# Skylarking/MARL

Measured on AMD Instinct MI355X. Metric: env_steps_per_sec, higher is better.
Workload: dtype f32 (bf16x6 split products, fp32 accumulate)

## Files before the change

### include/marl_hip.h

```cpp
#ifndef MARL_HIP_H
#define MARL_HIP_H
#include <stddef.h>
#ifdef __cplusplus
extern "C" {
#endif

typedef struct {
  const float* p0; long ld0; int k0;
  const float* p1; long ld1; int k1;
  const int* idx; int nhot; int hot_w;
  int nid;
  const float* m0; long ldm0;
  long rpe0, bs0, off0;
  long rpei, bsi, offi;
  const int* emap0;
} marl_src_t;

typedef struct {
  int groups;
  long gs_x0, gs_x1, gs_w, gs_b, gs_y, gs_m0;
} marl_group_t;

typedef struct {
  const float *fc1_w, *fc1_b;
  const float *w_ih, *w_hh;
  const float *b_ih, *b_hh;
  const float *fc2_w, *fc2_b;
  int H;
} marl_agent_weights_t;

int marl_linear(const marl_src_t* x, const float* W, long ldw, int w_kmajor, const float* bias,
                float* Y, long ldy, int M, int N, int K, int act, float beta,
                const marl_group_t* grp, void* stream);
int marl_linear_wgrad(const float* dY, long lddy, const float* Yact, long ldya, const marl_src_t* x,
                      float* dW, long lddw, float* db, int M, int N, int K, int flags,
                      const marl_group_t* grp, float* ws, size_t ws_bytes, void* stream);
size_t marl_linear_wgrad_workspace(int M, int N, int K, int groups);
int marl_wgrad_slabs(int M);

int marl_agent_unroll_fwd(const marl_agent_weights_t* w, const float* obs, long obs_bs, int obs_t0,
                          const int* ufed, long u_bs, int u_t0, const int* ep_len, const int* ep_map,
                          const float* h0, float* q, float* hs, float* h_last, float* saved, int B, int T,
                          int N, int O, int A, int last_action, int reuse_network, int cu_budget,
                          float* gi_out, const float* gi_in, void* stream);
int marl_agent_unroll_reuse_supported(int B, int T, int N, int O, int A, int cu_budget);

typedef struct {
  float *w_ih, *w_hh;
  float *b_ih, *b_hh;
  float *fc2_w, *fc2_b;
} marl_agent_grads_t;

size_t marl_agent_bwd_workspace(int B, int N, int A);
int marl_agent_unroll_bwd(const marl_agent_weights_t* w, const float* dq, const int* dq_idx,
                          const float* dq_val, const int* dq_idx2, const float* dq_val2, int dq_gdiv, const float* dhs,
                          const float* saved, const float* hs, float* dxp, float* dh0,
                          const marl_agent_grads_t* g, float* ws, size_t ws_bytes,
                          int B, int T, int N, int A, void* stream);

int marl_q_gather(const float* q, const int* idx, const float* avail, float mask_val, float* out,
                  long rows, int A, void* stream);
int marl_q_masked_max(const float* q, const float* avail, float mask_val, float* out_max, int* out_arg,
                      long rows, int A, void* stream);
int marl_q_double_select(const float* q_sel, const float* q_val, const float* avail, float mask_val,
                         float* out_val, int* out_arg, long rows, int A, void* stream);
int marl_q_scatter(float* dq, const int* idx1, const float* g1, const int* idx2, const float* g2,
                   long rows, int A, int gdiv, void* stream);
int marl_vec_add(const float* a, const float* b, float* out, long n, void* stream);
int marl_agent_sum(const float* in, long ld_in, float* out, long ld_out, long rows, int N, int D, void* stream);
int marl_agent_bcast(const float* in, long ld_in, float* out, long ld_out, long rows, int N, int D, int accumulate,
                     void* stream);

int marl_qmix_mix_fwd(const float* hy, long ldh, const float* b2, const float* w22, const float* b22, const float* q,
                      float* q_tot, long rows, int N, int E, void* stream);
int marl_qmix_mix_bwd(const float* hy, long ldh, const float* q, const float* dq_tot, const float* w22, float* dhy,
                      float* db2, float* dq, long rows, int N, int E, void* stream);
int marl_qmix_tail_fwd(const marl_src_t* s, long rows, int S, const float* Wb1, long ldb1, const float* bb1, const float* Wh,
                       long ldwh, const float* bh, float* hy, long ldhy, int c_b1, int c_h, void* stream);

typedef struct {
  const float *w1, *w1_b;
  const float *b1, *b1_b;
  const float *w2, *w2_b;
  const float *h, *h_b;
  const float *b2_w, *b2_b;
} marl_qmix_weights_t;
int marl_qmix_fused_supported(int N, int S, int E);
size_t marl_qmix_fused_workspace(long rows, int N, int S);
int marl_qmix_fused_fwd(const marl_qmix_weights_t* w, const marl_src_t* s, const float* q, float* q_tot,
                        long rows, int N, int S, int E, void* stream);
int marl_qmix_fused_bwd(const marl_qmix_weights_t* w, const marl_src_t* s, const float* q, const float* dq_tot,
                        float* dq, const marl_qmix_weights_t* grads, float* ws, size_t ws_bytes, long rows,
                        int N, int S, int E, void* stream);
int marl_qmix_fused_loss_bwd(const marl_qmix_weights_t* w, const marl_src_t* s, const float* q, const float* q_tot_tgt,
                             const float* r, const float* term, const float* padded, float gamma, float* q_tot,
                             float* dq, const marl_qmix_weights_t* grads, float* loss2, float* ws, size_t ws_bytes,
                             long rows, int N, int S, int E, void* stream);
int marl_qmix_fused_fwd_x6(const marl_qmix_weights_t* w, const marl_src_t* s, const float* q, float* q_tot,
                           long rows, int N, int S, int E, void* stream);
int marl_qmix_fused_bwd_x6(const marl_qmix_weights_t* w, const marl_src_t* s, const float* q, const float* dq_tot,
                           float* dq, const marl_qmix_weights_t* grads, float* ws, size_t ws_bytes, long rows,
                           int N, int S, int E, void* stream);
int marl_qmix_fused_loss_bwd_x6(const marl_qmix_weights_t* w, const marl_src_t* s, const float* q, const float* q_tot_tgt,
                                const float* r, const float* term, const float* padded, float gamma, float* q_tot,
                                float* dq, const marl_qmix_weights_t* grads, float* loss2, float* ws, size_t ws_bytes,
                                long rows, int N, int S, int E, void* stream);

int marl_qmix_wide_supported(int N, int S, int E);
const char* marl_qmix_wide_fwd_kernel(long rows, int N, int S, int flags);
size_t marl_qmix_wide_workspace(long rows, int N, int S, int backward);
int marl_qmix_wide_fwd(const marl_qmix_weights_t* w, const marl_src_t* s, const float* q, float* q_tot, float* ws,
                       size_t ws_bytes, long rows, int N, int S, int E, int flags, void* stream);
int marl_qmix_wide_bwd(const marl_qmix_weights_t* w, const marl_src_t* s, const float* q, const float* dq_tot, float* dq,
                       const marl_qmix_weights_t* grads, float* ws, size_t ws_bytes, long rows, int N, int S, int E,
                       int flags, void* stream);
int marl_qmix_wide_loss_bwd(const marl_qmix_weights_t* w, const marl_src_t* s, const float* q, const float* q_tot_tgt,
                            const float* r, const float* term, const float* padded, float gamma, float* q_tot, float* dq,
                            const marl_qmix_weights_t* grads, float* loss2, float* ws, size_t ws_bytes, long rows,
                            int N, int S, int E, int flags, void* stream);

typedef struct {
  const float *w1, *b1;
  const float *w2, *b2;
  const float *w3, *b3;
  long gs_w1, gs_b1, gs_w2, gs_b2, gs_w3, gs_b3;
} marl_mlp3_weights_t;
int marl_mlp3_supported(const marl_src_t* x, int K1, int H1, int H2, int N3, int groups);
int marl_mlp3_fwd(const marl_mlp3_weights_t* w, const marl_src_t* x, float* Y, long ldy, long gs_y,
                  long M, int K1, int N3, int groups, void* stream);
size_t marl_mlp3_bwd_workspace(long M, int K1, int N3, int groups);
int marl_mlp3_bwd(const marl_mlp3_weights_t* w, const marl_src_t* x, const float* dY, long lddy, long gs_dy,
                  const marl_mlp3_weights_t* grads, float* ws, size_t ws_bytes, long M, int K1, int N3,
                  int groups, void* stream);
size_t marl_mlp3_save_floats(long M, int three, int groups);
int marl_mlp3_needs_kept(const marl_src_t* x, int K1, int N3);
int marl_mlp3_fwd_save(const marl_mlp3_weights_t* w, const marl_src_t* x, float* Y, long ldy, long gs_y,
                       float* hsave, size_t hsave_floats, long M, int K1, int N3, int groups, void* stream);
int marl_mlp3_bwd_saved(const marl_mlp3_weights_t* w, const marl_src_t* x, const float* dY, long lddy, long gs_dy,
                        const marl_mlp3_weights_t* grads, float* ws, size_t ws_bytes, const float* hsave,
                        size_t hsave_floats, long M, int K1, int N3, int groups, void* stream);

int marl_agent_unroll_x6_supported(int B, int T, int N, int O, int A, int last_action, int reuse_network);
int marl_agent_unroll_x6_plain_r6(int B, int T, int N, int O, int A, int last_action, int reuse_network, int cu_budget);
int marl_agent_unroll_fwd_x6(const marl_agent_weights_t* w, const float* obs, long obs_bs, int obs_t0,
                             const int* ufed, long u_bs, int u_t0, const int* ep_len, const int* ep_map,
                             const float* h0, float* q, float* hs, float* h_last, float* saved, int B, int T, int N,
                             int O, int A, int last_action, int reuse_network, int cu_budget, float* gi_out,
                             const float* gi_in, void* stream);

#define MARL_UNROLL_SAVED 1
#define MARL_UNROLL_GI_OUT 2
#define MARL_UNROLL_GI_IN 4
#define MARL_UNROLL_HS 8
#define MARL_UNROLL_OBS_ALIGNED 16
#define MARL_UNROLL_H_ALIGNED 32
#define MARL_UNROLL_F32_PIPE 0
#define MARL_UNROLL_F32_MULTI 1
#define MARL_UNROLL_X6 2
#define MARL_UNROLL_X6_R6 3
#define MARL_UNROLL_IN_ELEMENT 0
#define MARL_UNROLL_IN_VECTOR 1
#define MARL_UNROLL_IN_HALF 2
#define MARL_UNROLL_IN_W2L 3
int marl_agent_unroll_fwd_plan(int x6, int B, int T, int N, int O, int A, int last_action, int reuse_network, int cu_budget,
                               int flags, int* plan);

int marl_agent_unroll_bwd_x6_supported(int B, int T, int N, int A, int sparse_dq);
size_t marl_agent_bwd_x6_workspace(int B, int N, int A);
int marl_agent_unroll_bwd_x6(const marl_agent_weights_t* w, const int* dq_idx, const float* dq_val, const int* dq_idx2,
                             const float* dq_val2, int dq_gdiv, const float* dhs, const float* saved, float* dxp, float* dh0,
                             const marl_agent_grads_t* g, float* ws, size_t ws_bytes, int B, int T, int N, int A, void* stream);

int marl_mlp3_x6_supported(const marl_src_t* x, int K1, int H1, int H2, int N3, int groups);
int marl_mlp3_x6_fwd_save(const marl_mlp3_weights_t* w, const marl_src_t* x, float* Y, long ldy, long gs_y,
                          float* hsave, size_t hsave_floats, long M, int K1, int N3, int groups, void* stream);
int marl_mlp3_x6_bwd_saved(const marl_mlp3_weights_t* w, const marl_src_t* x, const float* dY, long lddy, long gs_dy,
                           const marl_mlp3_weights_t* grads, float* ws, size_t ws_bytes, const float* hsave,
                           size_t hsave_floats, long M, int K1, int N3, int groups, void* stream);

typedef struct {
  const float *enc0_w, *enc0_b;
  const float *enc2_w, *enc2_b;
  const float* q0_w; long q0_ld; int q0_s;
  const float *q2_w, *q2_b;
  const float *q4_w, *q4_b;
} marl_qtran_weights_t;
int marl_qtran_supported(int N, int A, int AE);
int marl_qtran_head_fwd(const marl_qtran_weights_t* w, const float* hidden, const int* u, const float* sp, float* out,
                        float* s1, float* e2, float* y1, float* y2, long BT, int N, int A, int AE, void* stream);
int marl_qtran_head_fwd2(const marl_qtran_weights_t* w, const float* hidden, const int* u, const int* u2, const float* sp,
                         float* out, float* out2, float* s1, float* e2, float* y1, float* y2, long BT, int N, int A, int AE,
                         void* stream);
size_t marl_qtran_bwd_workspace(long BT, int AE);
int marl_qtran_head_bwd(const marl_qtran_weights_t* w, const float* hidden, const int* u, const float* d_out,
                        const float* y1, const float* y2, float* dy1, float* dy2, float* de2, float* dhidden,
                        int accumulate, float* d_enc0_w, float* d_enc0_b, float* d_enc2_b, float* ws, size_t ws_bytes,
                        long BT, int N, int A, int AE, void* stream);

int marl_qtran_state_parts_supported(int S);
int marl_qtran_state_parts(const marl_src_t* s, long BT, int S, int nsets, const float* W0, long ldw0, const float* b0, float* sp0,
                           const float* W1, long ldw1, const float* b1, float* sp1, void* stream);
int marl_qtran_wgrad_rows_supported(int S, int AE);
size_t marl_qtran_wgrad_rows_workspace(int S, int AE);
int marl_qtran_wgrad_rows(const marl_src_t* s, const float* s1, const float* e2, const float* y1, const float* y2,
                          const float* d_out, const float* dy1, const float* dy2, const float* de2, float* d_q0_w, long ld_q0,
                          float* d_q0_b, float* d_q2_w, float* d_q2_b, float* d_q4_w, float* d_q4_b, float* d_enc2_w, float* ws,
                          size_t ws_bytes, long BT, int S, int AE, void* stream);

int marl_qplex_mix_fwd(const float* w_raw, const float* v, const float* q, const float* max_q,
                       const float* key, const float* ag, const float* ac, float* v_tot, float* a_tot,
                       float* lam_out, long rows, int N, int K, int weighted_head, int minus_one,
                       void* stream);
int marl_qplex_mix_bwd(const float* w_raw, const float* q, const float* max_q, const float* key,
                       const float* ag, const float* ac, const float* g, float* dq, float* dw_raw,
                       float* dv, float* dkey, float* dag, float* dac, long rows, int N, int K,
                       int weighted_head, int minus_one, void* stream);

int marl_first_terminated_len(const float* term, long ld, int E, int T, int* out, void* stream);

int marl_replay_gather(const long long* idx, int B, int T, int N, int A, const int* u_src, const float* r_src,
                       const float* term_src, const float* padded_src, const int* length_src, const int* won_src,
                       const float* avail_src, int* o_map, int* u, int* u_act, float* r, float* term, float* padded,
                       int* length, int* won, float* avail_next, float* avail_cur, void* stream);

int marl_td_loss(const float* q_tot, const float* q_tot_tgt, const float* r, const float* term,
                 const float* padded, float gamma, float* dq_tot, float* out2, float* ws, long rows,
                 void* stream);
int marl_qtran_loss(const float* jq, const float* jq_tgt, const float* v, const float* jq_hat,
                    const float* qsum_opt, const float* qsum_nopt, const float* r, const float* term,
                    const float* padded, float gamma, float lam_opt, float lam_nopt, float* d_jq,
                    float* d_v, float* d_qsum_opt, float* d_qsum_nopt, float* out4, float* ws, long rows,
                    void* stream);
size_t marl_loss_workspace(long rows);

int marl_td_lambda_returns(const float* q_next_tot, const float* r, const float* term, const float* padded,
                           float gamma, float lambda, float* ret, int B, int T, void* stream);

int marl_policy_probs(const float* logits, const float* avail, float eps, float* pi, long rows, int A, void* stream);
int marl_policy_loss_bwd(const float* logits, const float* avail, const int* u, const float* G, const float* v,
                         const float* padded, float eps, float* dlogits, float* logp, float* out2, float* ws, long rows,
                         int N, int A, void* stream);
int marl_policy_loss_bwd_ex(const float* logits, const float* avail, const int* u, const float* G, const float* v,
                            const float* padded, float eps, float beta, float* dlogits, float* logp, float* ent, float* out3,
                            float* ws, long rows, int N, int A, void* stream);
int marl_policy_sample(const float* logits, const float* avail, long avail_es, const int* alive, float eps,
                       unsigned rseed, int env0, const int* tg, int tg0, int* act_out, long act_es,
                       int E, int N, int A, void* stream);

int marl_coma_onehot_cols(const float* W, long ldw, int col0, float* Wt, int C, int D, void* stream);
int marl_coma_fc1_fwd(const float* pre_s, const float* Wt, const int* u, float* h1, int B, int T, int N, int A, int D,
                      void* stream);
size_t marl_coma_fc1_bwd_workspace(int B, int T, int N, int A, int D);
int marl_coma_fc1_bwd(const float* dh1, const float* h1, const int* u, float* dpre, float* dsum, float* dW, long lddw,
                      int col0, float* ws, size_t ws_bytes, int B, int T, int N, int A, int D, void* stream);
int marl_coma_q_taken(const float* q, const int* u, float* out, int shift, int B, int T, int N, int A, void* stream);
int marl_coma_loss_bwd(const float* logits, const float* avail, const float* q, const int* u, const float* G,
                       const float* padded, float eps, float beta, float* dlogits, float* dq, float* logp, float* ent,
                       float* adv, float* q_taken, float* out_c2, float* out_a3, float* ws, int B, int T, int N, int A,
                       void* stream);

int marl_grad_sumsq(const float* g, long n, float* sumsq, float* ws, void* stream);
size_t marl_sumsq_workspace(long n);
int marl_rmsprop_step(float* p, const float* g, float* sq, long n, float lr, float alpha, float eps,
                      float clip, const float* sumsq, const float* den, void* stream);
int marl_adam_step(float* p, const float* g, float* m, float* v, long n, float lr, float beta1,
                   float beta2, float eps, float bc1, float bc2_sqrt, float clip, const float* sumsq,
                   const float* den, void* stream);

int marl_select_actions(const float* q, const float* avail, long avail_es, const int* alive, float eps,
                        unsigned rseed, int env0, const int* tg, int tg0, int* act_out, long act_es,
                        int E, int N, int A, void* stream);
int marl_synth_lengths(unsigned seed, int env0, int episode, int* len, int* won, int E, int T, void* stream);
int marl_synth_observe(unsigned seed, int env0, int episode, int t, const int* len, float* obs,
                       float* state, long state_ld, float* avail, int E, int T, int N, int O, int S, int A, void* stream);
int marl_synth_step(unsigned seed, int env0, int episode, int t, const int* len, const int* act,
                    int* u, float* r, float* term, float* padded, int* alive_next, int E, int T, int N, int A,
                    void* stream);

int marl_synth_fused_step(unsigned seed, unsigned rseed, int env0, int episode, int t, float eps, const int* len,
                          const float* q, float* obs, float* state, long state_ld, float* avail, int* u, float* r,
                          float* term, float* padded, int E, int T, int N, int O, int S, int A, void* stream);

int marl_synth_rollout_supported(int N, int O, int A);
int marl_synth_rollout(const marl_agent_weights_t* w, unsigned seed, unsigned rseed, int env0, int episode,
                       int fixed_len, const float* eps, float* obs, float* state, long state_ld, float* avail, int* u,
                       float* r, float* term, float* padded, int* length, int* won, float* h_out,
                       float* stats, double eps0, double eps_anneal, double eps_min, int E, int T, int N, int O, int S,
                       int A, int last_action, int reuse_network, void* stream);

int marl_synth_rollout_x6_supported_flags(int N, int O, int A, int last_action, int reuse_network);
int marl_synth_rollout_x6_supported(int N, int O, int A);
int marl_synth_rollout_x6_plan(int E, int N, int O, int A, int last_action, int reuse_network, int* plan);
int marl_synth_rollout_x6(const marl_agent_weights_t* w, unsigned seed, unsigned rseed, int env0, int episode,
                          int fixed_len, const float* eps, float* obs, float* state, long state_ld, float* avail, int* u,
                          float* r, float* term, float* padded, int* length, int* won, float* h_out,
                          float* stats, double eps0, double eps_anneal, double eps_min, int E, int T, int N, int O, int S,
                          int A, int last_action, int reuse_network, void* stream);

typedef struct {
  const float *t0_w, *t0_b, *t2_w, *t2_b;
  const float *w0_w, *w0_b, *w2_w, *w2_b;
  const float *wq_w, *wq_b, *wk_w, *wk_b;
  const float *v0_w, *v0_b, *v2_w, *v2_b;
} marl_rtw_weights_t;
int marl_rtw_supported(int N, int O, int A, int H, int hidden_dim, int attn_dim);
int marl_rtw_head_act(const marl_rtw_weights_t* w, const float* h, const float* obs, long obs_bs, int obs_t0,
                      const float* avail, long av_bs, int av_t0, float* q, int* a_out, float* ohat_out, int E, int N,
                      int O, int A, int not_self_model, void* stream);
int marl_rtw_head_given(const marl_rtw_weights_t* w, const float* hs, const float* obs, long obs_bs, int obs_t0,
                        const float* obs_next, long on_bs, int on_t0, const int* u, long u_bs, int u_t0, float* q,
                        int B, int T, int N, int O, int A, int not_self_model, void* stream);

typedef struct {
  const float *h0_w, *h0_b, *h2_w, *h2_b;
  const float *r_w, *r_b, *o_w, *o_b, *t_w, *t_b;
} marl_world_weights_t;
typedef struct {
  float *h0_w, *h0_b, *h2_w, *h2_b;
  float *r_w, *r_b, *o_w, *o_b;
} marl_world_grads_t;
int marl_world_supported(int N, int O, int A, int H);
size_t marl_world_fwd_workspace(int B, int T, int N);
int marl_world_head_fwd(const marl_world_weights_t* w, const float* h, float* q, float* r_out, float* ohat_out,
                        float* tau_out, const float* obs, long obs_bs, int obs_t0, const int* ep_len, const int* ep_map,
// ... 57 lines not shown
```

### marl_amd/_lib.py

```python
from __future__ import annotations

import ctypes as C
import os

_HERE = os.path.dirname(os.path.abspath(__file__))
LIB_PATH = os.environ.get("MARL_HIP_LIB") or os.path.join(_HERE, "libmarl_hip.so")

c_float_p = C.c_void_p
c_int_p = C.c_void_p


class MarlSrc(C.Structure):
    _fields_ = [("p0", C.c_void_p), ("ld0", C.c_long), ("k0", C.c_int),
                ("p1", C.c_void_p), ("ld1", C.c_long), ("k1", C.c_int),
                ("idx", C.c_void_p), ("nhot", C.c_int), ("hot_w", C.c_int),
                ("nid", C.c_int),
                ("m0", C.c_void_p), ("ldm0", C.c_long),
                ("rpe0", C.c_long), ("bs0", C.c_long), ("off0", C.c_long),
                ("rpei", C.c_long), ("bsi", C.c_long), ("offi", C.c_long),
                ("emap0", C.c_void_p)]


class MarlGroup(C.Structure):
    _fields_ = [("groups", C.c_int), ("gs_x0", C.c_long), ("gs_x1", C.c_long), ("gs_w", C.c_long),
                ("gs_b", C.c_long), ("gs_y", C.c_long), ("gs_m0", C.c_long)]


class MarlQmixWeights(C.Structure):
    _fields_ = [(n, C.c_void_p) for n in ("w1", "w1_b", "b1", "b1_b", "w2", "w2_b", "h", "h_b", "b2_w", "b2_b")]


class MarlMlp3Weights(C.Structure):
    _fields_ = ([(n, C.c_void_p) for n in ("w1", "b1", "w2", "b2", "w3", "b3")] +
                [(n, C.c_long) for n in ("gs_w1", "gs_b1", "gs_w2", "gs_b2", "gs_w3", "gs_b3")])


class MarlQtranWeights(C.Structure):
    _fields_ = [("enc0_w", C.c_void_p), ("enc0_b", C.c_void_p), ("enc2_w", C.c_void_p), ("enc2_b", C.c_void_p),
                ("q0_w", C.c_void_p), ("q0_ld", C.c_long), ("q0_s", C.c_int),
                ("q2_w", C.c_void_p), ("q2_b", C.c_void_p), ("q4_w", C.c_void_p), ("q4_b", C.c_void_p)]


class MarlRtwWeights(C.Structure):
    _fields_ = [(n, C.c_void_p) for n in ("t0_w", "t0_b", "t2_w", "t2_b", "w0_w", "w0_b", "w2_w", "w2_b",
                                          "wq_w", "wq_b", "wk_w", "wk_b", "v0_w", "v0_b", "v2_w", "v2_b")]


class MarlWorldWeights(C.Structure):
    _fields_ = [(n, C.c_void_p) for n in ("h0_w", "h0_b", "h2_w", "h2_b", "r_w", "r_b", "o_w", "o_b", "t_w", "t_b")]


class MarlWorldGrads(C.Structure):
    _fields_ = [(n, C.c_void_p) for n in ("h0_w", "h0_b", "h2_w", "h2_b", "r_w", "r_b", "o_w", "o_b")]


class MarlMaicWeights(C.Structure):
    _fields_ = [(n, C.c_void_p) for n in ("e0_w", "e0_b", "bn_w", "bn_b", "bn_rm", "bn_rv", "bn_nbt", "e3_w", "e3_b",
                                          "m0_w", "m0_b", "m2_w", "m2_b", "k_w", "k_b", "q_w", "q_b")]


class MarlMaicGrads(C.Structure):
    _fields_ = [(n, C.c_void_p) for n in ("e0_w", "e0_b", "bn_w", "bn_b", "e3_w", "e3_b", "m0_w", "m0_b", "m2_w", "m2_b",
                                          "k_w", "k_b", "q_w", "q_b")]


class MarlMaicInfer(C.Structure):
    _fields_ = [(n, C.c_void_p) for n in ("i0_w", "i0_b", "ibn_w", "ibn_b", "ibn_rm", "ibn_rv", "ibn_nbt", "i3_w", "i3_b")]


class MarlMaicInferGrads(C.Structure):
    _fields_ = [(n, C.c_void_p) for n in ("i0_w", "i0_b", "ibn_w", "ibn_b", "i3_w", "i3_b")]


class MarlAgentGrads(C.Structure):
    _fields_ = [("w_ih", C.c_void_p), ("w_hh", C.c_void_p), ("b_ih", C.c_void_p), ("b_hh", C.c_void_p),
                ("fc2_w", C.c_void_p), ("fc2_b", C.c_void_p)]


class MarlAgentWeights(C.Structure):
    _fields_ = [("fc1_w", C.c_void_p), ("fc1_b", C.c_void_p), ("w_ih", C.c_void_p), ("w_hh", C.c_void_p),
                ("b_ih", C.c_void_p), ("b_hh", C.c_void_p), ("fc2_w", C.c_void_p), ("fc2_b", C.c_void_p),
                ("H", C.c_int)]


P, I, L, F, U, SZ, D = C.c_void_p, C.c_int, C.c_long, C.c_float, C.c_uint, C.c_size_t, C.c_double
SRC, GRP, AW = C.POINTER(MarlSrc), C.POINTER(MarlGroup), C.POINTER(MarlAgentWeights)
AG = C.POINTER(MarlAgentGrads)
QW = C.POINTER(MarlQmixWeights)
M3 = C.POINTER(MarlMlp3Weights)
QT = C.POINTER(MarlQtranWeights)
RW = C.POINTER(MarlRtwWeights)
WW, WG = C.POINTER(MarlWorldWeights), C.POINTER(MarlWorldGrads)
MW, MG = C.POINTER(MarlMaicWeights), C.POINTER(MarlMaicGrads)
MIW, MIG = C.POINTER(MarlMaicInfer), C.POINTER(MarlMaicInferGrads)

SIGNATURES = {
    "marl_linear": (I, [SRC, P, L, I, P, P, L, I, I, I, I, F, GRP, P]),
    "marl_linear_wgrad": (I, [P, L, P, L, SRC, P, L, P, I, I, I, I, GRP, P, SZ, P]),
    "marl_linear_wgrad_workspace": (SZ, [I, I, I, I]),
    "marl_wgrad_slabs": (I, [I]),
    "marl_agent_unroll_fwd": (I, [AW, P, L, I, P, L, I, P, P, P, P, P, P, P, I, I, I, I, I, I, I, I, P, P, P]),
    "marl_agent_unroll_reuse_supported": (I, [I, I, I, I, I, I]),
    "marl_agent_unroll_x6_supported": (I, [I, I, I, I, I, I, I]),
    "marl_agent_unroll_x6_plain_r6": (I, [I, I, I, I, I, I, I, I]),
    "marl_agent_unroll_fwd_x6": (I, [AW, P, L, I, P, L, I, P, P, P, P, P, P, P, I, I, I, I, I, I, I, I, P, P, P]),
    "marl_agent_unroll_fwd_plan": (I, [I, I, I, I, I, I, I, I, I, I, P]),
    "marl_agent_bwd_workspace": (SZ, [I, I, I]),
    "marl_agent_unroll_bwd_x6_supported": (I, [I, I, I, I, I]),
    "marl_agent_bwd_x6_workspace": (SZ, [I, I, I]),
    "marl_agent_unroll_bwd_x6": (I, [AW, P, P, P, P, I, P, P, P, P, AG, P, SZ, I, I, I, I, P]),
    "marl_agent_unroll_bwd": (I, [AW, P, P, P, P, P, I, P, P, P, P, P, AG, P, SZ, I, I, I, I, P]),
    "marl_replay_gather": (I, [P, I, I, I, I] + [P] * 17 + [P]),
    "marl_q_gather": (I, [P, P, P, F, P, L, I, P]),
    "marl_q_masked_max": (I, [P, P, F, P, P, L, I, P]),
    "marl_q_double_select": (I, [P, P, P, F, P, P, L, I, P]),
    "marl_q_scatter": (I, [P, P, P, P, P, L, I, I, P]),
    "marl_vec_add": (I, [P, P, P, L, P]),
    "marl_agent_sum": (I, [P, L, P, L, L, I, I, P]),
    "marl_agent_bcast": (I, [P, L, P, L, L, I, I, I, P]),
    "marl_qmix_mix_fwd": (I, [P, L, P, P, P, P, P, L, I, I, P]),
    "marl_qmix_mix_bwd": (I, [P, L, P, P, P, P, P, P, L, I, I, P]),
    "marl_qmix_tail_fwd": (I, [SRC, L, I, P, L, P, P, L, P, P, L, I, I, P]),
    "marl_qmix_fused_supported": (I, [I, I, I]),
    "marl_qmix_fused_workspace": (SZ, [L, I, I]),
    "marl_qmix_fused_fwd": (I, [QW, SRC, P, P, L, I, I, I, P]),
    "marl_qmix_fused_bwd": (I, [QW, SRC, P, P, P, QW, P, SZ, L, I, I, I, P]),
    "marl_qmix_fused_loss_bwd": (I, [QW, SRC, P, P, P, P, P, F, P, P, QW, P, P, SZ, L, I, I, I, P]),
    "marl_qmix_fused_fwd_x6": (I, [QW, SRC, P, P, L, I, I, I, P]),
    "marl_qmix_fused_bwd_x6": (I, [QW, SRC, P, P, P, QW, P, SZ, L, I, I, I, P]),
    "marl_qmix_fused_loss_bwd_x6": (I, [QW, SRC, P, P, P, P, P, F, P, P, QW, P, P, SZ, L, I, I, I, P]),
    "marl_qmix_wide_supported": (I, [I, I, I]),
    "marl_qmix_wide_workspace": (SZ, [L, I, I, I]),
    "marl_qmix_wide_fwd_kernel": (C.c_char_p, [L, I, I, I]),
    "marl_qmix_wide_fwd": (I, [QW, SRC, P, P, P, SZ, L, I, I, I, I, P]),
    "marl_qmix_wide_bwd": (I, [QW, SRC, P, P, P, QW, P, SZ, L, I, I, I, I, P]),
    "marl_qmix_wide_loss_bwd": (I, [QW, SRC, P, P, P, P, P, F, P, P, QW, P, P, SZ, L, I, I, I, I, P]),
    "marl_mlp3_supported": (I, [SRC, I, I, I, I, I]),
    "marl_mlp3_fwd": (I, [M3, SRC, P, L, L, L, I, I, I, P]),
    "marl_mlp3_bwd_workspace": (SZ, [L, I, I, I]),
    "marl_mlp3_bwd": (I, [M3, SRC, P, L, L, M3, P, SZ, L, I, I, I, P]),
    "marl_mlp3_save_floats": (SZ, [L, I, I]),
    "marl_mlp3_needs_kept": (I, [SRC, I, I]),
    "marl_mlp3_fwd_save": (I, [M3, SRC, P, L, L, P, SZ, L, I, I, I, P]),
    "marl_mlp3_bwd_saved": (I, [M3, SRC, P, L, L, M3, P, SZ, P, SZ, L, I, I, I, P]),
    "marl_mlp3_x6_supported": (I, [SRC, I, I, I, I, I]),
    "marl_mlp3_x6_fwd_save": (I, [M3, SRC, P, L, L, P, SZ, L, I, I, I, P]),
    "marl_mlp3_x6_bwd_saved": (I, [M3, SRC, P, L, L, M3, P, SZ, P, SZ, L, I, I, I, P]),
    "marl_qtran_supported": (I, [I, I, I]),
    "marl_qtran_head_fwd": (I, [QT, P, P, P, P, P, P, P, P, L, I, I, I, P]),
    "marl_qtran_head_fwd2": (I, [QT, P, P, P, P, P, P, P, P, P, P, L, I, I, I, P]),
    "marl_qtran_bwd_workspace": (SZ, [L, I]),
    "marl_qtran_state_parts_supported": (I, [I]),
    "marl_qtran_state_parts": (I, [SRC, L, I, I, P, L, P, P, P, L, P, P, P]),
    "marl_qtran_wgrad_rows_supported": (I, [I, I]),
    "marl_qtran_wgrad_rows_workspace": (SZ, [I, I]),
    "marl_qtran_wgrad_rows": (I, [SRC] + [P] * 8 + [P, L, P, P, P, P, P, P, P, SZ, L, I, I, P]),
    "marl_qtran_head_bwd": (I, [QT, P, P, P, P, P, P, P, P, P, I, P, P, P, P, SZ, L, I, I, I, P]),
    "marl_qplex_mix_fwd": (I, [P, P, P, P, P, P, P, P, P, P, L, I, I, I, I, P]),
    "marl_qplex_mix_bwd": (I, [P, P, P, P, P, P, P, P, P, P, P, P, P, L, I, I, I, I, P]),
    "marl_first_terminated_len": (I, [P, L, I, I, P, P]),
    "marl_td_loss": (I, [P, P, P, P, P, F, P, P, P, L, P]),
    "marl_qtran_loss": (I, [P, P, P, P, P, P, P, P, P, F, F, F, P, P, P, P, P, P, L, P]),
    "marl_loss_workspace": (SZ, [L]),
    "marl_td_lambda_returns": (I, [P, P, P, P, F, F, P, I, I, P]),
    "marl_policy_probs": (I, [P, P, F, P, L, I, P]),
    "marl_policy_loss_bwd": (I, [P, P, P, P, P, P, F, P, P, P, P, L, I, I, P]),
    "marl_policy_loss_bwd_ex": (I, [P, P, P, P, P, P, F, F, P, P, P, P, P, L, I, I, P]),
    "marl_policy_sample": (I, [P, P, L, P, F, U, I, P, I, P, L, I, I, I, P]),
    "marl_coma_onehot_cols": (I, [P, L, I, P, I, I, P]),
    "marl_coma_fc1_fwd": (I, [P, P, P, P, I, I, I, I, I, P]),
    "marl_coma_fc1_bwd_workspace": (SZ, [I, I, I, I, I]),
    "marl_coma_fc1_bwd": (I, [P, P, P, P, P, P, L, I, P, SZ, I, I, I, I, I, P]),
    "marl_coma_q_taken": (I, [P, P, P, I, I, I, I, I, P]),
    "marl_coma_loss_bwd": (I, [P, P, P, P, P, P, F, F, P, P, P, P, P, P, P, P, P, I, I, I, I, P]),
    "marl_grad_sumsq": (I, [P, L, P, P, P]),
    "marl_sumsq_workspace": (SZ, [L]),
    "marl_rmsprop_step": (I, [P, P, P, L, F, F, F, F, P, P, P]),
    "marl_adam_step": (I, [P, P, P, P, L, F, F, F, F, F, F, F, P, P, P]),
    "marl_select_actions": (I, [P, P, L, P, F, U, I, P, I, P, L, I, I, I, P]),
    "marl_synth_lengths": (I, [U, I, I, P, P, I, I, P]),
    "marl_synth_observe": (I, [U, I, I, I, P, P, P, L, P, I, I, I, I, I, I, P]),
    "marl_synth_step": (I, [U, I, I, I, P, P, P, P, P, P, P, I, I, I, I, P]),
    "marl_synth_fused_step": (I, [U, U, I, I, I, F, P, P, P, P, L, P, P, P, P, P, I, I, I, I, I, I, P]),
    "marl_synth_rollout_supported": (I, [I, I, I]),
    "marl_synth_rollout": (I, [AW, U, U, I, I, I, P, P, P, L, P, P, P, P, P, P, P, P, P, D, D, D, I, I, I, I, I, I, I, I, P]),
    "marl_synth_rollout_x6_supported": (I, [I, I, I]),
    "marl_synth_rollout_x6_supported_flags": (I, [I, I, I, I, I]),
    "marl_synth_rollout_x6_plan": (I, [I, I, I, I, I, I, P]),
    "marl_synth_rollout_x6": (I, [AW, U, U, I, I, I, P, P, P, L, P, P, P, P, P, P, P, P, P, D, D, D, I, I, I, I, I, I, I, I, P]),
    "marl_rtw_supported": (I, [I, I, I, I, I, I]),
    "marl_rtw_head_act": (I, [RW, P, P, L, I, P, L, I, P, P, P, I, I, I, I, I, P]),
    "marl_rtw_head_given": (I, [RW, P, P, L, I, P, L, I, P, L, I, P, I, I, I, I, I, I, P]),
    "marl_world_supported": (I, [I, I, I, I]),
    "marl_world_fwd_workspace": (SZ, [I, I, I]),
    "marl_world_head_fwd": (I, [WW, P, P, P, P, P, P, L, I, P, P, P, P, SZ, I, I, I, I, I, P]),
    "marl_world_bwd_workspace": (SZ, [I, I, I, I, I]),
    "marl_world_head_bwd": (I, [WW, WG, P, P, P, P, L, I, P, P, P, F, P, P, SZ, I, I, I, I, I, P]),
    "marl_maic_supported": (I, [I, I, I, I, I, I, I]),
    "marl_maic_workspace": (SZ, [I, I]),
    "marl_maic_head_fwd": (I, [MW, P, P, P, P, P, P, P, P, P, SZ, I, I, I, I, I, F, F, F, P]),
    "marl_maic_noise": (I, [U, I, U, P, I, I, P]),
    "marl_maic_bwd_workspace": (SZ, [I, I, I]),
    "marl_maic_head_bwd": (I, [MW, MG, P, P, P, P, P, P, SZ, I, I, I, I, I, F, F, P]),
    "marl_maic_head_bwd_ex": (I, [MW, MG, P, P, P, P, P, P, P, SZ, I, I, I, I, I, F, F, P]),
    "marl_maic_aux_workspace": (SZ, [I, I, I]),
    "marl_maic_aux": (I, [MW, MIW, MG, MIG, P, P, P, F, F, P, F, P, P, P, P, P, SZ, I, I, I, I, I, F, F, F, P]),
    "marl_hip_version": (C.c_char_p, []),
    "marl_experiment_set": (I, [C.c_char_p, I]),
    "marl_experiment_get": (I, [C.c_char_p]),
}

_lib = None


class MarlHipError(RuntimeError):
    pass


def load():
    global _lib
    if _lib is not None:
        return _lib
    if not os.path.exists(LIB_PATH):
        raise MarlHipError(
            "libmarl_hip.so not found at %s - the HIP hot path is mandatory (no CPU fallback). "
            "Build it with `python -c \"import __graft_entry__ as g; g.build()\"`." % LIB_PATH)
    lib = C.CDLL(LIB_PATH)
    for name, (res, args) in SIGNATURES.items():
        fn = getattr(lib, name)
        fn.restype = res
        fn.argtypes = args
    _lib = lib
    from . import experiments
    experiments.apply(lib)
    return lib


def check(code, what):
    if code != 0:
        raise MarlHipError("%s failed with hipError_t %d" % (what, code))
```

### marl_amd/algorithm/common.py

```python
from __future__ import annotations

import copy
import numbers
import os
import warnings
import weakref

import numpy as np
import torch

from .. import ops, experiments
from ..hostutil import FlatParams, DeviceBatch, AsyncInt, require_cuda
from ..network.mixer import x6_mode
from ..rollout import EpisodeBatch

MASK_BIG = -9999999.0
MASK_QTRAN_EVAL = -999999.0
N_STATS = 4


class FlatView:

    def __init__(self, flat, params, start):
        self.params = list(params)
# ... 134 lines not shown
    _full_len_streak = 0
    n_stats, den_slot = 2, 1
    extra_nets = ()
    launch_ahead = True
    replay_graphs = True

    def _begin(self, mac, args, name):
        self.td_lambda = td_lambda_of(args)
        self._td_dbg = {}
        self.max_episode_len = args.episode_limit
        self.gamma = args.gamma
        self.lr = args.lr
        self.model_dir = args.model_dir + '/' + args.alg + '/' + args.map
        self.args = args
        self.device = require_cuda(name)

        self.eval_net = mac
        self.eval_net.cuda()
        self.target_net = copy.deepcopy(mac)

    def _ready(self, needs_avail):
        args = self.args
        self.optimizer = FusedOptimizer(self._flat, args.optimizer, self.lr, args.grad_norm_clip)
        self._buf = Scratch()
        self.reducer = GradReducer()
        self.pair = PairedUnroll(x6=x6_mode(args))
        self.loss_readback = LossReadback(args)
        self.graphs = GraphedUpdate.from_args(args) if self.replay_graphs else None
        self.needs_avail = needs_avail
        self.last_stats = None
        self.sync_replicas()

    def _update_targets(self):
        self.target_net.agent._flat.flat.copy_(self.eval_net.agent._flat.flat)
        if self.mixer is not None and self.mixer._flat.n:
            self.target_mixer._flat.flat.copy_(self.mixer._flat.flat)

    def _g(self, name, shape, dt=torch.float32):
        return self._buf.get(name, shape, self.device, dt)

    def _td_inputs(self, db, q_next_tot):
        lam = self.td_lambda = td_lambda_of(self.args)
        if lam is None:
            self._td_dbg = {}
            return db.r, self.gamma
        G = self._g("td_ret", (db.B * db.T,))
        ops.td_lambda_returns(q_next_tot, db.r, db.term, db.padded, self.gamma, lam, G, db.B, db.T)
        self._td_dbg = {"td_targets": G}
        return G, 0.0

    def get_max_episode_len(self, batch):
        T = DeviceBatch.first_terminated_len(torch.as_tensor(np.asarray(batch['terminated'])), self.args.episode_limit)
        for key in batch.keys():
            batch[key] = batch[key][:, :T]
        return batch, T

    def _device_batch(self, rec, index, small):
        term = (small if small is not None else rec).term
        if not (term.is_cuda and term.dtype == torch.float32 and term.shape[0] > 0) or self._full_len_streak < 2 \
                or not self.launch_ahead:
            db = DeviceBatch.from_record_auto(rec, self.args, reducer=self.reducer, index=index, small=small)
            full = db.T == min(rec.T, self.args.episode_limit)
            self._full_len_streak = self._full_len_streak + 1 if full else 0
            return db
        db, pending = DeviceBatch.from_record_begin(rec, self.args, reducer=self.reducer, index=index, small=small)
        self.max_episode_len = db.T
        self._forward_backward(db)
        T = pending()
        if T == db.T:
            return None
        self._full_len_streak = 0
        return DeviceBatch.from_record(rec, self.args, T=T, index=index, small=small)

    def train(self, batch, train_step):
        ring = batch.ring if isinstance(batch, EpisodeBatch) else None
        if self.graphs is not None and ring is not None and self.graphs.run(self, ring, batch.index):
            db = None
        elif isinstance(batch, DeviceBatch):
            db = batch
        elif ring is not None:
            prep = self.graphs.prepared if self.graphs is not None else None
            if prep is not None:
                self.graphs.prepared = None
                db = DeviceBatch.from_record(ring, self.args, T=prep[1], index=batch.index, small=prep[0])
            else:
                small = ring.select_small(batch.index, avail_cur=self.needs_avail)
                db = self._device_batch(ring, batch.index, small)
        elif isinstance(batch, EpisodeBatch) and batch.record is not None:
            db = self._device_batch(batch.record, None, None)
        else:
            T = None
            if self.reducer.enabled:
                T = DeviceBatch.first_terminated_len(torch.as_tensor(np.asarray(batch['terminated'])),
                                                     self.args.episode_limit, reducer=self.reducer)
            db = DeviceBatch.from_dict(batch, self.args, self.device, T=T)
        if db is not None:
            self.max_episode_len = db.T
            self._forward_backward(db)
        return self._finish_update(train_step)

    def _loss_fn(self):
        return lambda s: s[0] / s[1]

    def _finish_update(self, train_step):
        self.reducer.allreduce_(self._flat.gradx)
        stats = self._flat.stats
        self.optimizer.step(den=stats[self.den_slot:self.den_slot + 1])
        if train_step > 0 and train_step % self.args.target_update_cycle == 0:
            self._update_targets()
        self.last_stats = stats
        return self.loss_readback.read(stats[:self.n_stats], self._loss_fn())

    def save_models(self, train_step):
        num = str(train_step // self.args.save_cycle)
        if not os.path.exists(self.model_dir):
            os.makedirs(self.model_dir)
        self.eval_net.save_models(self.model_dir + '/' + num + '_rnn_net_params.pkl')
        for name in ("mixer",) + self.extra_nets:
            torch.save({k: v.detach().cpu() for k, v in getattr(self, name).state_dict().items()},
                       self.model_dir + '/' + num + '_' + name + '_net_params.pkl')

    def load_models(self):
        if os.path.exists(self.model_dir + '/rnn_net_params.pkl'):
            path_rnn = self.model_dir + '/rnn_net_params.pkl'
            path_mix = self.model_dir + '/mixer_net_params.pkl'
            self.eval_net.load_models(path_rnn)
            for name in ("mixer",) + self.extra_nets:
                getattr(self, name).load_state_dict(torch.load(self.model_dir + '/' + name + '_net_params.pkl', map_location='cpu'))
            self.sync_replicas()
            print('Successfully load the model: {} and {}'.format(path_rnn, path_mix))
        else:
            raise Exception("No model!")


class Scratch:
    def __init__(self):
        self.d = {}

    def get(self, name, shape, device, dtype=torch.float32):
        key = (name, tuple(shape), dtype)
        t = self.d.get(key)
        if t is None or t.device != device:
            t = torch.empty(*shape, dtype=dtype, device=device)
            self.d[key] = t
        return t


def agent_backward(mac, db, which, saved, hs, dq, dhs, buf, dq_idx=None, dq_val=None, dq_idx2=None, dq_val2=None, dq_gdiv=1):
    args = mac.args
    B, T, N, A, O = db.B, db.T, db.N, db.A, db.O
    H = args.rnn_hidden_dim
    M = B * T * N
    dev = saved.device
    dxp = buf.get("dxp", (B, T, N, H), dev)
    w = mac.agent.weights()
    ag = mac.agent
    grads = {"rnn.weight_ih": ag.rnn.weight_ih.grad, "rnn.weight_hh": ag.rnn.weight_hh.grad,
             "rnn.bias_ih": ag.rnn.bias_ih.grad, "rnn.bias_hh": ag.rnn.bias_hh.grad,
             "fc2.weight": ag.fc2.weight.grad, "fc2.bias": ag.fc2.bias.grad}
    x6 = (x6_mode(args) and dq is None and dq_idx is not None
          and (B * N + 31) // 32 >= experiments.get("x6_bwd_min_wg") and ops.agent_unroll_bwd_x6_supported(B, T, N, A))
    ops.agent_unroll_bwd(w, dq, dhs, saved, hs, dxp, None, grads, B, T, N, A, dq_idx=dq_idx, dq_val=dq_val,
                         dq_idx2=dq_idx2, dq_val2=dq_val2, dq_gdiv=dq_gdiv, x6=x6)
    obs, obs_bs, obs_t0 = db.o_cur if which == "cur" else db.o_next
    remap0 = None if (obs_bs == T * N and obs_t0 == 0) else (T * N, obs_bs, obs_t0 * N)
    kw = {}
    if args.last_action:
        kw.update(idx=db.u_fed.reshape(-1, 1), nhot=1, hot_w=A, remapi=(T * N, db.u_bs, (-1 if which == "cur" else 0) * N))
    emap = getattr(db, 'o_map', None)
    if emap is not None and remap0 is None:
        remap0 = (T * N, obs_bs, obs_t0 * N)
    xin = ops.src(obs.reshape(-1, O), nid=N if args.reuse_network else 0, remap0=remap0, emap0=emap, **kw)
    I = O + (A if args.last_action else 0) + (N if args.reuse_network else 0)
    ops.linear_wgrad(dxp.view(M, H), xin, ag.fc1.weight.grad, ag.fc1.bias.grad, M, H, I, bf16=False)


class GradReducer:

    def __init__(self, group=None):
        import torch.distributed as dist
        self.dist = dist
        self.group = group
        up = dist.is_available() and dist.is_initialized()
        self.enabled = up and (dist.get_world_size(group) > 1 or experiments.get("force_reducer") == 1)

    def allreduce_(self, flat_with_stats):
        if self.enabled:
            self.dist.all_reduce(flat_with_stats, op=self.dist.ReduceOp.SUM, group=self.group)
        return flat_with_stats

    def broadcast_(self, *tensors, src=0):
        if self.enabled:
            for t in tensors:
                if t is not None:
                    self.dist.broadcast(t, src=src, group=self.group)

    def max_int(self, value, device):
        if not self.enabled:
            return value
        t = torch.tensor([value], dtype=torch.int64, device=device)
        self.dist.all_reduce(t, op=self.dist.ReduceOp.MAX, group=self.group)
        return int(t.item())


class PairedUnroll:

    MAX_TILES = 1024

    def __init__(self, x6=False):
        self.side = None
        self.x6 = bool(x6)
        self.enabled = experiments.get("no_pair") != 1
        self.chain = experiments.get("no_chain") != 1
        self.forced_split = experiments.get("chain_split")

    def applies(self, rows, T):
        return self.enabled and T >= 8 and 32 <= (rows + 15) // 16 <= self.MAX_TILES

    def run(self, rows, T, first, second):
        if not self.applies(rows, T):
            first(256)
            second(256)
            return
        self._fork(lambda: first(128), lambda: second(128))

    def _fork(self, main, side):
        cur = torch.cuda.current_stream()
        if self.side is None or self.side.device != cur.device:
            self.side = torch.cuda.Stream(device=cur.device)
        self.side.wait_stream(cur)
        with torch.cuda.stream(self.side):
            side()
        main()
        cur.wait_stream(self.side)

    def _step_us(self, rt):
        if self.x6:
            return 1.5 if rt <= 1 else 2.75 if rt <= 2 else 1.74 * rt
        return 3.3 if rt <= 1 else 1.3 + 2.1 * rt

    def chain_split(self, rows, T, obs_dim):
        if not self.chain or not self.applies(rows, T):
            return None
        if self.forced_split is not None:
            return (self.forced_split, 256 - self.forced_split) if self.forced_split > 0 else None
        tiles = (rows + 15) // 16
        cap = 8 if self.x6 else max(1, min(8, 2048 // (4 * max(obs_dim, 4))))
        ceil = lambda a, b: -(-a // b)
        plain = self._step_us(ceil(tiles, 128)) + 0.6 * self._step_us(ceil(tiles, 256))
        best = None
        for cu_a in (128, 144, 160, 176, 192):
            cu_b = 256 - cu_a
            rt_a, rt_b = ceil(tiles, cu_a), ceil(tiles, cu_b)
            if rt_a > cap or rt_b > cap:
                continue
            cost = max(1.6 * self._step_us(rt_a), self._step_us(rt_b))
            if best is None or cost < best[0]:
                best = (cost, cu_a, cu_b)
        if best is None or best[0] > 0.9 * plain:
            return None
        return best[1], best[2]

    def run_chain(self, rows, T, obs_dim, first, cont, second):
        split = self.chain_split(rows, T, obs_dim) if cont is not None else None
        if split is None:
            self.run(rows, T, first, second)
            if cont is not None:
                cont(256)
            return
        cu_a, cu_b = split
        self._fork(lambda: (first(cu_a), cont(cu_a)), lambda: second(cu_b))


class GraphedUpdate:

    WARMUP = 2
    AUTO_MAX_EPISODES = 1536

    def __init__(self, auto=False):
        self.entries = {}
        self.disabled = False
        self.auto = bool(auto)
        self.replays = 0

    @staticmethod
    def from_args(args):
        mode = getattr(args, "hip_graph", None)
        if mode is None or mode == "auto":
            return GraphedUpdate(auto=True)
        return GraphedUpdate() if mode else None

    SCHEDULE_ARGS = ("gemm_mode", "mixer_dtype", "mixer_wgrad_dtype", "double_q", "no_loss_fold", "lazy_loss", "gamma",
                     "two_hyper_layers", "last_action", "reuse_network", "td_lambda")

    @staticmethod
    def _schedule_key(args):
        return (experiments.generation,) + tuple(repr(getattr(args, k, None)) for k in GraphedUpdate.SCHEDULE_ARGS)

    def run(self, learner, ring, index):
        self.prepared = None
        if self.disabled:
            return False
        args = learner.args
        if self.auto and int(index.numel()) > self.AUTO_MAX_EPISODES:
            return False
        if ring.T != args.episode_limit or int(index.numel()) != int(args.batch_size):
            return False
        key = (id(ring), int(index.numel()), ring.T)
        e = self.entries.get(key)
        if e is not None and e["ring"]() is not ring:
            e = None
        dev = ring.obs.device
        if e is None:
            idx = index.to(device=dev, dtype=torch.long).clone()
            small = ring.select_small(idx, avail_cur=getattr(learner, "needs_avail", False))
            db = DeviceBatch.from_record(ring, args, T=min(ring.T, args.episode_limit), index=idx, small=small)
            fused = getattr(small, "avail_next", None) is not None and db.T == ring.T
            e = self.entries[key] = dict(ring=weakref.ref(ring), idx=idx, small=small, db=db, calls=0, graph=None, streak=0,
                                         fused=fused, avail_next=None if fused else db.avail_next.clone(),
                                         u_act=None if fused else db.u_act.clone())
            if not fused:
                db.avail_next, db.u_act = e["avail_next"], e["u_act"]
            e["T"] = db.T
        idx, small, db = e["idx"], e["small"], e["db"]
        idx.copy_(index)
        db.o_map.copy_(idx)
# ... 56 lines not shown
```

### marl_amd/csrc/agent_bwd_x6.hip

```cpp
#include "x6.h"
#include <cstdlib>
#include "../../include/marl_hip.h"

#ifndef DWHH_HEAD
#define DWHH_HEAD -1
#endif
namespace {

constexpr int H = 64;
constexpr int BNT = 512;
constexpr int GPL = 256 * 64;
constexpr int GBUF = 3 * GPL;
constexpr int FRB = 4 * 3 * 1024;

struct BX6Args {
  const float *Wih, *Whh, *W2;
  const int* dq_idx; const float* dq_val;
  const int* dq_idx2; const float* dq_val2;
  int dq_gdiv;
  const float* dhs;
  const float* saved;
  float* dxp;
  float* dh0;
  float* ws;
  int B, T, N, A;
  long R;
  long tile_base;
  int slab_base;
};

__host__ __device__ inline long slab_floats(int A) { return 2L * 192 * 64 + (long)A * 64 + 2 * 192 + A; }

#define X6_TERMS4(A0, B0, A1, B1, c0, c1, c2, c3)                                                                   \
  c0 = mm(A0.m, B0.m, c0); c1 = mm(A1.m, B1.m, c1); c2 = mm(A0.h, B0.m, c2); c3 = mm(A1.h, B1.m, c3);               \
  c0 = mm(A0.h, B0.l, c0); c1 = mm(A1.h, B1.l, c1); c2 = mm(A0.m, B0.h, c2); c3 = mm(A1.m, B1.h, c3);               \
  c0 = mm(A0.l, B0.h, c0); c1 = mm(A1.l, B1.h, c1); c2 = mm(A0.h, B0.h, c2); c3 = mm(A1.h, B1.h, c3);

__device__ __forceinline__ long sv_off(long tile_t, int plane, int c, int lane) { return ((tile_t * 6 + plane) * 4 + c) * 256 + lane * 4; }

__device__ __forceinline__ F3 wTfrag(const float* W, int c, int u0, int lane) {
  const int j = lane & 15, g = lane >> 4;
  float v[8];
#pragma unroll
  for (int jj = 0; jj < 8; ++jj) v[jj] = W[(long)(32 * c + 8 * g + jj) * H + u0 + j];
  return split8((f32x4){v[0], v[1], v[2], v[3]}, (f32x4){v[4], v[5], v[6], v[7]});
}
__device__ __forceinline__ i32x4 g_tr(const char* img, int tb0, int tb1, int off, int tile) {
  typedef __attribute__((address_space(3))) s16x4 lds_s16x4;
  const s16x4 lo = __builtin_amdgcn_ds_read_tr16_b64_v4i16((lds_s16x4*)(img + off + (tb0 ^ (32 * tile))));
  const s16x4 hi = __builtin_amdgcn_ds_read_tr16_b64_v4i16((lds_s16x4*)(img + off + (tb1 ^ (32 * tile))));
  return __builtin_bit_cast(i32x4, (s16x8)__builtin_shufflevector(lo, hi, 0, 1, 2, 3, 4, 5, 6, 7));
}
__device__ __forceinline__ F3 g_tr3(const char* img, int tb0, int tb1, int k0, int tile) {
  F3 f;
  f.h = g_tr(img, tb0, tb1, k0 * 64, tile); f.m = g_tr(img, tb0, tb1, k0 * 64 + GPL, tile); f.l = g_tr(img, tb0, tb1, k0 * 64 + 2 * GPL, tile);
  return f;
}
__device__ __forceinline__ F3 g_cols(const char* img, int rb, int k0) {
  F3 f;
  const char* p = img + k0 * 64;
#pragma unroll
  for (int pl = 0; pl < 3; ++pl) {
    const i32x2 t0 = *reinterpret_cast<const i32x2*>(p + pl * GPL + rb);
    const i32x2 t1 = *reinterpret_cast<const i32x2*>(p + pl * GPL + (rb ^ 32));
    const i32x4 v = (i32x4){t0[0], t0[1], t1[0], t1[1]};
    if (pl == 0) f.h = v; else if (pl == 1) f.m = v; else f.l = v;
  }
  return f;
}
__device__ __forceinline__ void g_put(char* img, int wb, int k0, int tile, const F3h& f) {
  char* p = img + k0 * 64 + (wb ^ (32 * tile));
  *reinterpret_cast<i32x2*>(p) = f.h;
  *reinterpret_cast<i32x2*>(p + GPL) = f.m;
  *reinterpret_cast<i32x2*>(p + 2 * GPL) = f.l;
}
__device__ __forceinline__ void fr_put(char* fr, int tile, int lane, const F3& f) {
  i32x4* p = reinterpret_cast<i32x4*>(fr) + tile * 192 + lane;
  p[0] = f.h; p[64] = f.m; p[128] = f.l;
}
__device__ __forceinline__ F3 fr_get(const char* fr, int tile, int lane) {
  const i32x4* p = reinterpret_cast<const i32x4*>(fr) + tile * 192 + lane;
  F3 f;
  f.h = p[0]; f.m = p[64]; f.l = p[128];
  return f;
}

template <int NT> struct FW;
template <> struct FW<2> { typedef F3 T; };
template <> struct FW<1> { typedef F3h T; };
__device__ __forceinline__ f32x4 mmx(const i32x4& a, const i32x4& b, f32x4 c) { return mm(a, b, c); }
__device__ __forceinline__ f32x4 mmx(const i32x2& a, const i32x2& b, f32x4 c) { return mmh(a, b, c); }
__device__ __forceinline__ void mm6x(const F3& a, const F3& b, f32x4& c) { mm6(a, b, c); }
__device__ __forceinline__ void mm6x(const F3h& a, const F3h& b, f32x4& c) { mm6h(a, b, c); }
__device__ __forceinline__ void fr_put(char* fr, int tile, int lane, const F3h& f) {
  i32x2* p = reinterpret_cast<i32x2*>(fr) + tile * 192 + lane;
  p[0] = f.h; p[64] = f.m; p[128] = f.l;
}
template <int NT> __device__ __forceinline__ typename FW<NT>::T fr_getn(const char* fr, int tile, int lane);
template <> __device__ __forceinline__ F3 fr_getn<2>(const char* fr, int tile, int lane) { return fr_get(fr, tile, lane); }
template <> __device__ __forceinline__ F3h fr_getn<1>(const char* fr, int tile, int lane) {
  const i32x2* p = reinterpret_cast<const i32x2*>(fr) + tile * 192 + lane;
  F3h f;
  f.h = p[0]; f.m = p[64]; f.l = p[128];
  return f;
}
template <int NT> __device__ __forceinline__ typename FW<NT>::T g_colsn(const char* img, int rb, int k0);
template <> __device__ __forceinline__ F3 g_colsn<2>(const char* img, int rb, int k0) { return g_cols(img, rb, k0); }
template <> __device__ __forceinline__ F3h g_colsn<1>(const char* img, int rb, int k0) {
  const char* p = img + k0 * 64 + rb;
  F3h f;
  f.h = *reinterpret_cast<const i32x2*>(p); f.m = *reinterpret_cast<const i32x2*>(p + GPL); f.l = *reinterpret_cast<const i32x2*>(p + 2 * GPL);
  return f;
}
__device__ __forceinline__ F3 splitn(const f32x4 (&x)[2]) { return split8(x[0], x[1]); }
__device__ __forceinline__ F3h splitn(const f32x4 (&x)[1]) { return split4(x[0]); }

template <bool DHS, bool TWO, int NT>
__global__ __launch_bounds__(BNT, 2) void agent_bwd_x6_kernel(BX6Args a) {
  typedef typename FW<NT>::T FWT;
  extern __shared__ __attribute__((aligned(16))) char smem[];
  const int tid = threadIdx.x, lane = tid & 63, wave = __builtin_amdgcn_readfirstlane(tid >> 6);
  const int team = wave >> 2, s = wave & 3;
  const int q = lane >> 4, m = lane & 15, u = 16 * s + m;
  char* Gt = smem;
  char* WL = Gt + GBUF;
  char* HB = WL + 4 * FRB;
  char* XB = HB + 2 * FRB;
  float* W2s = reinterpret_cast<float*>(XB + 2 * FRB);
  int4* QT = reinterpret_cast<int4*>(W2s + 32 * H);
  int* rowidx = reinterpret_cast<int*>(QT + 3 * 32);
  int* rowrho = rowidx + 32;
  unsigned* XM = reinterpret_cast<unsigned*>(rowrho + 32);
  float* BS = reinterpret_cast<float*>(XM + 512);

  const long NTILES = (a.R + 15) >> 4;
  const long tile0 = (long)NT * blockIdx.x + a.tile_base;
  const long tl[2] = {tile0, tile0 + 1 < NTILES ? tile0 + 1 : tile0};
  if (tid < 16 * NT) {
    const long rho = tile0 * 16 + tid;
    const bool ok = rho < a.R;
    rowidx[tid] = ok ? (int)((rho / a.N) * a.T * a.N + rho % a.N) : -1;
    rowrho[tid] = ok ? (int)rho : -1;
  }
  for (int e = tid; e < 32 * H; e += BNT) W2s[e] = e < a.A * H ? a.W2[e] : 0.f;
  __syncthreads();
  const int T = a.T;
  auto qraw = [&](int r, int t) {
    int4 e = make_int4(-1, 0, -1, 0);
    const int ri = rowidx[r];
    if (ri >= 0 && t >= 0) {
      const unsigned k = (unsigned)ri + (unsigned)t * (unsigned)a.N;
      const unsigned kv = a.dq_gdiv == 1 ? k : k / (unsigned)a.dq_gdiv;
      e.x = a.dq_idx[k];
      e.y = __float_as_int(a.dq_val[kv]);
      if (a.dq_idx2) { e.z = a.dq_idx2[k]; e.w = __float_as_int(a.dq_val2[kv]); }
    }
    return e;
  };
  constexpr bool QDR = NT == 1;
  auto qfix = [&](int4 e) {
    const bool ok1 = e.x >= 0 && e.x < a.A, ok2 = e.z >= 0 && e.z < a.A;
    return make_int4(ok1 ? e.x : 0, ok1 ? e.y : 0, ok2 ? e.z : 0, ok2 ? e.w : 0);
  };
  auto lane_parts = [&](int& wb_, int& tb0_, int& tb1_) {
    int l = lane;
    asm volatile("" : "+v"(l));
    const int q_ = l >> 4, m_ = l & 15, qq = m_ >> 2, p4 = m_ & 3;
    wb_ = m_ * 64 + 8 * (q_ ^ (2 * ((m_ >> 2) & 3)));
    tb0_ = (8 * q_ + qq) * 64 + 8 * (p4 ^ (2 * ((2 * q_) & 3)));
    tb1_ = (8 * q_ + 4 + qq) * 64 + 8 * (p4 ^ (2 * ((2 * q_ + 1) & 3)));
  };
  ST_DECL(4);
  if (team == 0) {
    F3 whT[4], wiT[4];
#pragma unroll
    for (int c = 0; c < 4; ++c) { whT[c] = wTfrag(a.Whh, c, 16 * s, lane); wiT[c] = wTfrag(a.Wih, c, 16 * s, lane); }
    char* wl = WL + s * FRB;
    fr_put(wl, 0, lane, wTfrag(a.Whh, 4, 16 * s, lane)); fr_put(wl, 1, lane, wTfrag(a.Whh, 5, 16 * s, lane));
    fr_put(wl, 2, lane, wTfrag(a.Wih, 4, 16 * s, lane)); fr_put(wl, 3, lane, wTfrag(a.Wih, 5, 16 * s, lane));
    f32x4 carry[NT];
#pragma unroll
    for (int tt = 0; tt < NT; ++tt) carry[tt] = splat(0.f);
    constexpr bool BSL = DHS || NT == 1;
    float* bsl = BS + tid;
    float bsr[4] = {0.f, 0.f, 0.f, 0.f};
    if (BSL) {
#pragma unroll
      for (int k = 0; k < 4; ++k) bsl[256 * k] = 0.f;
    }
    f32x4 sv[NT][5];
    f32x4 dhsv[NT];
    auto svload = [&](int t, int tt) {
      const float* sp = a.saved + sv_off((long)t * NTILES + tl[tt], 0, s, lane);
      sv[tt][0] = *reinterpret_cast<const f32x4*>(sp);
      sv[tt][1] = *reinterpret_cast<const f32x4*>(sp + 2 * 1024);
      sv[tt][2] = *reinterpret_cast<const f32x4*>(sp + 3 * 1024);
      sv[tt][3] = *reinterpret_cast<const f32x4*>(sp + 4 * 1024);
      sv[tt][4] = *reinterpret_cast<const f32x4*>(sp + 5 * 1024);
      if (DHS) {
#pragma unroll
        for (int r = 0; r < 4; ++r) {
          const int ri = rowidx[16 * tt + 4 * q + r];
          dhsv[tt][r] = ri >= 0 ? a.dhs[(unsigned)(ri + t * a.N) * (unsigned)H + (unsigned)u] : 0.f;
        }
      }
    };
    svload(T - 1, 0);
    if (NT == 2) svload(T - 1, NT - 1);
    if (tid < 16 * NT) { QT[((T - 1) % 3) * 32 + tid] = qfix(qraw(tid, T - 1)); QT[((T - 2 + 3) % 3) * 32 + tid] = qfix(qraw(tid, T - 2)); }
    int4 qnR = make_int4(-1, 0, -1, 0);
    if (QDR && tid < 16 * NT) qnR = qraw(tid, T - 3);
    __syncthreads();
    for (int t = T - 1; t >= 0; --t) {
      const int par = t & 1;
      char* img = Gt;
      const int4* qt = QT + (t % 3) * 32;
      int wb, tb0, tb1;
      lane_parts(wb, tb0, tb1);
#pragma unroll
      for (int tt = 0; tt < NT; ++tt) {
        f32x4 drp, dzp, dnp, dhn;
#pragma unroll
        for (int r = 0; r < 4; ++r) {
          const int4 e = qt[16 * tt + 4 * q + r];
          float dh = carry[tt][r];
          if (DHS) dh += dhsv[tt][r];
          dh = __fmaf_rn(__int_as_float(e.y), W2s[e.x * H + u], dh);
          if (TWO) dh = __fmaf_rn(__int_as_float(e.w), W2s[e.z * H + u], dh);
          const float hp = sv[tt][0][r], rg = sv[tt][1][r], zg = sv[tt][2][r], ng = sv[tt][3][r], hn = sv[tt][4][r];
          const float dn = dh * (1.f - zg);
          const float dz = dh * (hp - ng);
          carry[tt][r] = dh * zg;
          const float dnp_ = dn * (1.f - ng * ng);
          const float dr = dnp_ * hn;
          dnp[r] = dnp_;
          dhn[r] = dnp_ * rg;
          drp[r] = dr * rg * (1.f - rg);
          dzp[r] = dz * zg * (1.f - zg);
        }
        const float s0 = (drp[0] + drp[1]) + (drp[2] + drp[3]), s1 = (dzp[0] + dzp[1]) + (dzp[2] + dzp[3]);
        const float s2 = (dnp[0] + dnp[1]) + (dnp[2] + dnp[3]), s3 = (dhn[0] + dhn[1]) + (dhn[2] + dhn[3]);
        if (BSL) { bsl[0] += s0; bsl[256] += s1; bsl[512] += s2; bsl[768] += s3; }
        else { bsr[0] += s0; bsr[1] += s1; bsr[2] += s2; bsr[3] += s3; }
        g_put(img, wb, 0 * 64 + 16 * s, tt, split4(drp));
        g_put(img, wb, 1 * 64 + 16 * s, tt, split4(dzp));
        g_put(img, wb, 2 * 64 + 16 * s, tt, split4(dnp));
        g_put(img, wb, 3 * 64 + 16 * s, tt, split4(dhn));
      }
      if (QDR && tid < 16 * NT) {
        if (t >= 2) QT[((t - 2) % 3) * 32 + tid] = qfix(qnR);
        qnR = qraw(tid, t - 3);
      }
      ST_MARK(0);
      WG_BARRIER();
      ST_MARK(1);
      __builtin_amdgcn_sched_barrier(0);
      if (t > 0) { svload(t - 1, 0); if (NT == 2) svload(t - 1, NT - 1); }
      const unsigned xmask = XM[par * 256 + s * 64 + lane];
      __builtin_amdgcn_sched_barrier(0);
#pragma unroll
      for (int tt = 0; tt < NT; ++tt) {
        f32x4 ca = carry[tt], cb = splat(0.f), da = splat(0.f), db = splat(0.f);
#pragma unroll
        for (int cp = 0; cp < 2; ++cp) {
          const F3 a0 = g_tr3(img, tb0, tb1, 64 * cp, tt), a1 = g_tr3(img, tb0, tb1, 64 * cp + 32, tt);
#define OP(p_, q_) ca = mm(a0.p_, whT[2 * cp].q_, ca); cb = mm(a1.p_, whT[2 * cp + 1].q_, cb); da = mm(a0.p_, wiT[2 * cp].q_, da); db = mm(a1.p_, wiT[2 * cp + 1].q_, db);
          X6_TERMS(OP)
#undef OP
          __builtin_amdgcn_sched_barrier(0);
        }
        {
          const F3 a0 = g_tr3(img, tb0, tb1, 192, tt), a1 = g_tr3(img, tb0, tb1, 192 + 32, tt);
          const F3 w4 = fr_get(wl, 0, lane), w5 = fr_get(wl, 1, lane);
#define OP(p_, q_) ca = mm(a0.p_, w4.q_, ca); cb = mm(a1.p_, w5.q_, cb);
          X6_TERMS(OP)
#undef OP
        }
        carry[tt] = ca + cb;
        __builtin_amdgcn_sched_barrier(0);
        {
          const F3 a0 = g_tr3(img, tb0, tb1, 128, tt), a1 = g_tr3(img, tb0, tb1, 128 + 32, tt);
          const F3 w4 = fr_get(wl, 2, lane), w5 = fr_get(wl, 3, lane);
#define OP(p_, q_) da = mm(a0.p_, w4.q_, da); db = mm(a1.p_, w5.q_, db);
          X6_TERMS(OP)
#undef OP
        }
        __builtin_amdgcn_sched_barrier(0);
        const f32x4 dx = da + db;
#pragma unroll
        for (int r = 0; r < 4; ++r) {
          const int ri = rowidx[16 * tt + 4 * q + r];
          if (ri >= 0) a.dxp[(unsigned)(ri + t * a.N) * (unsigned)H + (unsigned)u] = (xmask >> (4 * tt + r)) & 1u ? dx[r] : 0.f;
        }
      }
      __builtin_amdgcn_sched_barrier(0);
      ST_MARK(2);
      WG_BARRIER();
      ST_MARK(3);
    }
    ST_DUMP(4);
    if (a.dh0) {
#pragma unroll
      for (int tt = 0; tt < NT; ++tt)
#pragma unroll
        for (int r = 0; r < 4; ++r) {
          const int rho = rowrho[16 * tt + 4 * q + r];
          if (rho >= 0) a.dh0[(long)rho * H + u] = carry[tt][r];
        }
    }
    float* slab = a.ws + ((long)blockIdx.x + a.slab_base) * slab_floats(a.A);
    float bs[4];
#pragma unroll
    for (int k = 0; k < 4; ++k) {
      bs[k] = BSL ? bsl[256 * k] : bsr[k];
      bs[k] += __shfl_xor(bs[k], 16);
      bs[k] += __shfl_xor(bs[k], 32);
    }
    if (q == 0) {
      float* db = slab + 2 * 192 * 64 + (long)a.A * H;
      db[0 * 64 + u] = bs[0]; db[1 * 64 + u] = bs[1]; db[2 * 64 + u] = bs[2];
      db[192 + 0 * 64 + u] = bs[0]; db[192 + 1 * 64 + u] = bs[1]; db[192 + 2 * 64 + u] = bs[3];
    }
  } else {
    const int ti = tid - 256;
    f32x4 accI[3][4], accH[3][4], acc2[2] = {splat(0.f), splat(0.f)};
#pragma unroll
    for (int b = 0; b < 3; ++b)
#pragma unroll
      for (int c = 0; c < 4; ++c) { accI[b][c] = splat(0.f); accH[b][c] = splat(0.f); }
    float bs2[2] = {0.f, 0.f};
    f32x4 xn[NT], hn[NT];
    auto xhload = [&](int t) {
#pragma unroll
      for (int tt = 0; tt < NT; ++tt) {
        const float* sp = a.saved + sv_off((long)t * NTILES + tl[tt], 0, s, lane);
        hn[tt] = *reinterpret_cast<const f32x4*>(sp);
        xn[tt] = *reinterpret_cast<const f32x4*>(sp + 1024);
      }
    };
    auto publish = [&](int t) {
      fr_put(XB + (t & 1) * FRB, s, lane, splitn(xn));
      fr_put(HB + (t & 1) * FRB, s, lane, splitn(hn));
      unsigned mk = 0;
#pragma unroll
      for (int tt = 0; tt < NT; ++tt)
#pragma unroll
        for (int r = 0; r < 4; ++r) mk |= xn[tt][r] > 0.f ? 1u << (4 * tt + r) : 0u;
      XM[(t & 1) * 256 + s * 64 + lane] = mk;
    };
    auto dw2 = [&](const int4* qt, const FWT& hb) {
#pragma unroll
      for (int ac = 0; ac < 2; ++ac) {
        if (ac == 1 && a.A <= 16) break;
        const int col = 16 * ac + m;
        f32x4 d[NT];
        float sum = 0.f;
#pragma unroll
        for (int tt = 0; tt < NT; ++tt) {
#pragma unroll
          for (int r = 0; r < 4; ++r) {
            const int4 e = qt[16 * tt + 4 * q + r];
            d[tt][r] = (e.x == col ? __int_as_float(e.y) : 0.f) + (TWO && e.z == col ? __int_as_float(e.w) : 0.f);
          }
          sum += (d[tt][0] + d[tt][1]) + (d[tt][2] + d[tt][3]);
        }
        bs2[ac] += sum;
        mm6x(splitn(d), hb, acc2[ac]);
      }
    };
    xhload(T - 1);
    publish(T - 1);
    xhload(T - 2);
    int4 qn = make_int4(-1, 0, -1, 0);
    if (!QDR && ti < 16 * NT) qn = qraw(ti, T - 3);
    __syncthreads();
    {
      f32x4 hT[NT];
#pragma unroll
      for (int tt = 0; tt < NT; ++tt) hT[tt] = *reinterpret_cast<const f32x4*>(a.saved + sv_off((long)T * NTILES + tl[tt], 0, s, lane));
      dw2(QT + ((T - 1) % 3) * 32, splitn(hT));
    }
    for (int t = T - 1; t >= 0; --t) {
      const int par = t & 1;
      const char* img = Gt;
      WG_BARRIER();
      ST_MARK(0);
      if (!QDR && ti < 16 * NT) {
        if (t >= 2) QT[((t - 2) % 3) * 32 + ti] = qfix(qn);
        qn = qraw(ti, t - 3);
      }
      int rb, tb0, tb1;
      lane_parts(rb, tb0, tb1);
      const FWT ar = g_colsn<NT>(img, rb, 0 * 64 + 16 * s), az = g_colsn<NT>(img, rb, 1 * 64 + 16 * s);
      const FWT ani = g_colsn<NT>(img, rb, 2 * 64 + 16 * s), anh = g_colsn<NT>(img, rb, 3 * 64 + 16 * s);
      if (t > 0) publish(t - 1);
      if (t > 1) xhload(t - 2);
      __builtin_amdgcn_sched_barrier(0);
#pragma unroll
      for (int c = 0; c < 4; ++c) {
        const FWT xb = fr_getn<NT>(XB + par * FRB, c, lane);
#define OP(p_, q_) accI[0][c] = mmx(ar.p_, xb.q_, accI[0][c]); accI[1][c] = mmx(az.p_, xb.q_, accI[1][c]); accI[2][c] = mmx(ani.p_, xb.q_, accI[2][c]);
        X6_TERMS(OP)
#undef OP
      }
      constexpr int HEAD = DWHH_HEAD >= 0 ? DWHH_HEAD : (NT == 2 ? 1 : 0);
#pragma unroll
      for (int c = 0; c < HEAD; ++c) {
        const FWT hb = fr_getn<NT>(HB + par * FRB, c, lane);
#define OP(p_, q_) accH[0][c] = mmx(ar.p_, hb.q_, accH[0][c]); accH[1][c] = mmx(az.p_, hb.q_, accH[1][c]); accH[2][c] = mmx(anh.p_, hb.q_, accH[2][c]);
        X6_TERMS(OP)
#undef OP
      }
      __builtin_amdgcn_sched_barrier(0);
      ST_MARK(1);
      WG_BARRIER();
      ST_MARK(2);
#pragma unroll
      for (int c = HEAD; c < 4; ++c) {
        const FWT hb = fr_getn<NT>(HB + par * FRB, c, lane);
#define OP(p_, q_) accH[0][c] = mmx(ar.p_, hb.q_, accH[0][c]); accH[1][c] = mmx(az.p_, hb.q_, accH[1][c]); accH[2][c] = mmx(anh.p_, hb.q_, accH[2][c]);
        X6_TERMS(OP)
#undef OP
      }
      __builtin_amdgcn_sched_barrier(0);
      if (t > 0) dw2(QT + ((t - 1) % 3) * 32, fr_getn<NT>(HB + par * FRB, s, lane));
      ST_MARK(3);
    }
    ST_DUMP(4);
    float* slab = a.ws + ((long)blockIdx.x + a.slab_base) * slab_floats(a.A);
#pragma unroll
    for (int b = 0; b < 3; ++b)
#pragma unroll
      for (int c = 0; c < 4; ++c)
#pragma unroll
        for (int r = 0; r < 4; ++r) {
          slab[(long)(64 * b + 16 * s + 4 * q + r) * H + 16 * c + m] = accI[b][c][r];
          slab[192 * 64 + (long)(64 * b + 16 * s + 4 * q + r) * H + 16 * c + m] = accH[b][c][r];
        }
#pragma unroll
    for (int ac = 0; ac < 2; ++ac) {
#pragma unroll
      for (int r = 0; r < 4; ++r)
        if (16 * ac + 4 * q + r < a.A) slab[2 * 192 * 64 + (long)(16 * ac + 4 * q + r) * H + u] = acc2[ac][r];
      float b = bs2[ac];
      b += __shfl_xor(b, 16);
      b += __shfl_xor(b, 32);
      if (s == 0 && q == 0 && 16 * ac + m < a.A) slab[2 * 192 * 64 + (long)a.A * H + 2 * 192 + 16 * ac + m] = b;
    }
  }
}

struct RedArgs {
  const float* ws; int nwg; int A;
  float *dWih, *dWhh, *dW2, *dbih, *dbhh, *db2;
};
constexpr int BRSG = 16;
__global__ __launch_bounds__(64 * BRSG) void agent_bwd_x6_reduce_kernel(RedArgs a) {
  __shared__ float part[BRSG][64];
  const long slab = slab_floats(a.A);
  const int el = threadIdx.x & 63, sg = threadIdx.x >> 6;
  const long e = (long)blockIdx.x * 64 + el;
  float s = 0.f;
  if (e < slab) s = slab_sum(a.ws + e, slab, sg, BRSG, a.nwg);
  part[sg][el] = s;
  __syncthreads();
  if (sg != 0 || e >= slab) return;
  s = 0.f;
#pragma unroll
  for (int g = 0; g < BRSG; ++g) s += part[g][el];
  long k = e;
  if (k < 192 * 64) { a.dWih[k] += s; return; }
  k -= 192 * 64;
  if (k < 192 * 64) { a.dWhh[k] += s; return; }
  k -= 192 * 64;
  if (k < (long)a.A * 64) { a.dW2[k] += s; return; }
  k -= (long)a.A * 64;
  if (k < 192) { a.dbih[k] += s; return; }
  k -= 192;
  if (k < 192) { a.dbhh[k] += s; return; }
  k -= 192;
  a.db2[k] += s;
}

}

extern "C" int marl_agent_unroll_bwd_x6_supported(int B, int T, int N, int A, int sparse_dq) {
  if (B < 1 || T < 3 || N < 1 || A < 1 || A > 32 || !sparse_dq) return 0;
  if ((double)B * T * N * H * 4.0 >= 4294967296.0) return 0;
  return 1;
}

static void bx6_plan(long R, long& n2, long& n1) {
  const long tiles = (R + 15) / 16;
  if (tiles <= 256) { n2 = 0; n1 = tiles; return; }
  n2 = tiles / 512 * 256;
  const long rem = tiles - 2 * n2;
  if (n2 > 0 && rem > 0 && rem <= 256) { n1 = rem; return; }
  n2 = (tiles + 1) / 2; n1 = 0;
}

extern "C" size_t marl_agent_bwd_x6_workspace(int B, int N, int A) {
  long n2, n1;
  bx6_plan((long)B * N, n2, n1);
  return (size_t)(n2 + n1) * slab_floats(A) * sizeof(float);
}

extern "C" int marl_agent_unroll_bwd_x6(const marl_agent_weights_t* w, const int* dq_idx, const float* dq_val, const int* dq_idx2,
                                        const float* dq_val2, int dq_gdiv, const float* dhs, const float* saved, float* dxp,
                                        float* dh0, const marl_agent_grads_t* g, float* ws, size_t ws_bytes, int B, int T, int N,
                                        int A, void* stream) {
  if (B <= 0 || T <= 0) return 0;
  if (w->H != H || !marl_agent_unroll_bwd_x6_supported(B, T, N, A, dq_idx != nullptr) || !dq_val || (dq_idx2 && !dq_val2))
    return (int)hipErrorInvalidValue;
  if (ws_bytes < marl_agent_bwd_x6_workspace(B, N, A) || (reinterpret_cast<uintptr_t>(saved) & 15)) return (int)hipErrorInvalidValue;
  BX6Args a;
  a.Wih = w->w_ih; a.Whh = w->w_hh; a.W2 = w->fc2_w;
  a.dq_idx = dq_idx; a.dq_val = dq_val; a.dq_idx2 = dq_idx2; a.dq_val2 = dq_val2; a.dq_gdiv = dq_gdiv > 1 ? dq_gdiv : 1;
  a.dhs = dhs; a.saved = saved; a.dxp = dxp; a.dh0 = dh0; a.ws = ws;
  a.B = B; a.T = T; a.N = N; a.A = A; a.R = (long)B * N;
  long n2, n1;
  bx6_plan(a.R, n2, n1);
  const size_t lds = (size_t)GBUF + 8 * FRB + 32 * H * 4 + 3 * 32 * 16 + 2 * 32 * 4 + 2 * 256 * 4 + 4 * 256 * 4;
#define BX6_PICK(NT_) (dhs ? (dq_idx2 ? (const void*)agent_bwd_x6_kernel<true, true, NT_> : (const void*)agent_bwd_x6_kernel<true, false, NT_>) \
                           : (dq_idx2 ? (const void*)agent_bwd_x6_kernel<false, true, NT_> : (const void*)agent_bwd_x6_kernel<false, false, NT_>))
  hipStream_t st = (hipStream_t)stream;
  for (int pass = 0; pass < 2; ++pass) {
    const long nwg = pass == 0 ? n2 : n1;
    if (nwg == 0) continue;
    const void* fn = pass == 0 ? BX6_PICK(2) : BX6_PICK(1);
    a.tile_base = pass == 0 ? 0 : 2 * n2;
    a.slab_base = pass == 0 ? 0 : (int)n2;
    hipError_t e = hipFuncSetAttribute(fn, hipFuncAttributeMaxDynamicSharedMemorySize, (int)lds);
    if (e != hipSuccess) return (int)e;
    void* kargs[] = {(void*)&a};
    e = hipLaunchKernel(fn, dim3((unsigned)nwg), dim3(BNT), kargs, lds, st);
    if (e != hipSuccess) return (int)e;
    MARL_CHECK_LAUNCH();
  }
#undef BX6_PICK
  RedArgs r;
  r.ws = ws; r.nwg = (int)(n2 + n1); r.A = A;
  r.dWih = g->w_ih; r.dWhh = g->w_hh; r.dW2 = g->fc2_w; r.dbih = g->b_ih; r.dbhh = g->b_hh; r.db2 = g->fc2_b;
  const long slab = slab_floats(A);
  hipLaunchKernelGGL(agent_bwd_x6_reduce_kernel, dim3((unsigned)((slab + 63) / 64)), dim3(64 * BRSG), 0, st, r);
  MARL_CHECK_LAUNCH();
  return 0;
}

ST_DEFINE_SETTER(marl_debug_stamps_agent_bwd_x6)
```

### marl_amd/csrc/common.h

```cpp
#pragma once
#include <hip/hip_runtime.h>
#include <stdint.h>

#define MARL_WAVE 64

#define WG_BARRIER() asm volatile("s_waitcnt lgkmcnt(0)\n\ts_barrier" ::: "memory")

struct MarlSwitches {
  int fwd_xs, fwd_w2l, bwd_pipe_max_rt, wgrad_tall, wide_res, rollout_v1, unroll_r6;
};
extern "C" const MarlSwitches* marl_switches(void);

#ifndef MARL_PAD_H
#define MARL_PAD_H 8
#endif
#ifndef MARL_PAD_K
#define MARL_PAD_K 8
#endif
#ifndef MARL_PAD_G
#define MARL_PAD_G 8
#endif

typedef float f32x4 __attribute__((ext_vector_type(4)));
typedef int i32x4 __attribute__((ext_vector_type(4)));

__device__ __forceinline__ f32x4 mfma16(float a, float b, f32x4 c) {
  return __builtin_amdgcn_mfma_f32_16x16x4f32(a, b, c, 0, 0, 0);
}

__device__ __forceinline__ f32x4 mfma16x4(const f32x4& a, const f32x4& b, f32x4 c) {
  c = mfma16(a[0], b[0], c);
  c = mfma16(a[1], b[1], c);
  c = mfma16(a[2], b[2], c);
  c = mfma16(a[3], b[3], c);
  return c;
}

#ifdef MARL_NO_INTERLEAVE
__device__ __forceinline__ void mfma16x4_il2(const f32x4& a0, const f32x4& b0, f32x4& c0, const f32x4& a1, const f32x4& b1, f32x4& c1) {
  c0 = mfma16x4(a0, b0, c0); c1 = mfma16x4(a1, b1, c1);
}
__device__ __forceinline__ void mfma16x4_il3(const f32x4& a0, const f32x4& b0, f32x4& c0, const f32x4& a1, const f32x4& b1, f32x4& c1,
                                             const f32x4& a2, const f32x4& b2, f32x4& c2) {
  c0 = mfma16x4(a0, b0, c0); c1 = mfma16x4(a1, b1, c1); c2 = mfma16x4(a2, b2, c2);
}
__device__ __forceinline__ void mfma16x4_il4(const f32x4& a0, const f32x4& b0, f32x4& c0, const f32x4& a1, const f32x4& b1, f32x4& c1,
                                             const f32x4& a2, const f32x4& b2, f32x4& c2, const f32x4& a3, const f32x4& b3, f32x4& c3) {
  c0 = mfma16x4(a0, b0, c0); c1 = mfma16x4(a1, b1, c1); c2 = mfma16x4(a2, b2, c2); c3 = mfma16x4(a3, b3, c3);
}
#else
__device__ __forceinline__ void mfma16x4_il2(const f32x4& a0, const f32x4& b0, f32x4& c0, const f32x4& a1, const f32x4& b1, f32x4& c1) {
#pragma unroll
  for (int i = 0; i < 4; ++i) { c0 = mfma16(a0[i], b0[i], c0); c1 = mfma16(a1[i], b1[i], c1); }
}
__device__ __forceinline__ void mfma16x4_il3(const f32x4& a0, const f32x4& b0, f32x4& c0, const f32x4& a1, const f32x4& b1, f32x4& c1,
                                             const f32x4& a2, const f32x4& b2, f32x4& c2) {
#pragma unroll
  for (int i = 0; i < 4; ++i) { c0 = mfma16(a0[i], b0[i], c0); c1 = mfma16(a1[i], b1[i], c1); c2 = mfma16(a2[i], b2[i], c2); }
}
__device__ __forceinline__ void mfma16x4_il4(const f32x4& a0, const f32x4& b0, f32x4& c0, const f32x4& a1, const f32x4& b1, f32x4& c1,
                                             const f32x4& a2, const f32x4& b2, f32x4& c2, const f32x4& a3, const f32x4& b3, f32x4& c3) {
#pragma unroll
  for (int i = 0; i < 4; ++i) {
    c0 = mfma16(a0[i], b0[i], c0); c1 = mfma16(a1[i], b1[i], c1); c2 = mfma16(a2[i], b2[i], c2); c3 = mfma16(a3[i], b3[i], c3);
  }
}

#endif

typedef short s16x4 __attribute__((ext_vector_type(4)));
typedef __bf16 bf16x4_t __attribute__((ext_vector_type(4)));
__device__ __forceinline__ f32x4 mfma16x4_bf16(const f32x4& a, const f32x4& b, f32x4 c) {
  const s16x4 ab = __builtin_bit_cast(s16x4, __builtin_convertvector(a, bf16x4_t));
  const s16x4 bb = __builtin_bit_cast(s16x4, __builtin_convertvector(b, bf16x4_t));
  return __builtin_amdgcn_mfma_f32_16x16x16bf16_1k(ab, bb, c, 0, 0, 0);
}
template <bool BF>
__device__ __forceinline__ f32x4 mm16x4(const f32x4& a, const f32x4& b, f32x4 c) {
  if (BF) return mfma16x4_bf16(a, b, c);
  return mfma16x4(a, b, c);
}

__device__ __forceinline__ float sigmoidf_(float x) { return __builtin_amdgcn_rcpf(1.0f + __expf(-x)); }
__device__ __forceinline__ float tanhf_(float x) {
  float e = __expf(2.0f * x);
  return 1.0f - 2.0f * __builtin_amdgcn_rcpf(e + 1.0f);
}

#define MARL_NLOG2E (-1.4426950408889634f)
#define MARL_2LOG2E (2.8853900817779268f)
#define MARL_INV_2LOG2E (0.34657359027997264f)
__device__ __forceinline__ void gru_point_plain(float ar, float az, float ain, float ahn, float hp, float& r, float& z, float& n, float& h) {
  r = sigmoidf_(ar); z = sigmoidf_(az);
  n = tanhf_(ain + r * ahn);
  h = (1.f - z) * n + z * hp;
}
#ifdef MARL_NO_PRESCALE
#undef MARL_INV_2LOG2E
#define MARL_INV_2LOG2E (1.0f)
__device__ __forceinline__ void gru_prescale(f32x4 (&)[3][4], f32x4 (&)[3][4], float&, float&, float&, float&) {}
__device__ __forceinline__ void gru_point(float ar, float az, float ain, float ahn, float hp, float& r, float& z, float& n, float& h) {
  gru_point_plain(ar, az, ain, ahn, hp, r, z, n, h);
}
#else
__device__ __forceinline__ void gru_prescale(f32x4 (&wih)[3][4], f32x4 (&whh)[3][4], float& b_r, float& b_z, float& b_in, float& b_hn) {
#pragma unroll
  for (int c = 0; c < 4; ++c) {
    wih[0][c] *= MARL_NLOG2E; whh[0][c] *= MARL_NLOG2E;
    wih[1][c] *= MARL_NLOG2E; whh[1][c] *= MARL_NLOG2E;
    wih[2][c] *= MARL_2LOG2E; whh[2][c] *= MARL_2LOG2E;
  }
  b_r *= MARL_NLOG2E; b_z *= MARL_NLOG2E; b_in *= MARL_2LOG2E; b_hn *= MARL_2LOG2E;
}
__device__ __forceinline__ void gru_point(float ar, float az, float ain, float ahn, float hp, float& r, float& z, float& n, float& h) {
  r = __builtin_amdgcn_rcpf(1.0f + __builtin_amdgcn_exp2f(ar));
  z = __builtin_amdgcn_rcpf(1.0f + __builtin_amdgcn_exp2f(az));
  const float e = __builtin_amdgcn_exp2f(__builtin_fmaf(r, ahn, ain));
  n = __builtin_fmaf(-2.0f, __builtin_amdgcn_rcpf(e + 1.0f), 1.0f);
  h = __builtin_fmaf(z, hp - n, n);
}
#endif

__device__ __forceinline__ float slab_acc(float s, const float* p, long stride, int w0, int step, int n) {
  int w = w0;
  for (; w + 7 * step < n; w += 8 * step) {
    float v[8];
#pragma unroll
    for (int u = 0; u < 8; ++u) v[u] = p[(long)(w + u * step) * stride];
#pragma unroll
    for (int u = 0; u < 8; ++u) s += v[u];
  }
  for (; w < n; w += step) s += p[(long)w * stride];
  return s;
}
__device__ __forceinline__ float slab_sum(const float* p, long stride, int w0, int step, int n) { return slab_acc(0.f, p, stride, w0, step, n); }

__device__ __forceinline__ float wave_sum(float v) {
#pragma unroll
  for (int o = 32; o > 0; o >>= 1) v += __shfl_xor(v, o, 64);
  return v;
}

template <int CTRL>
__device__ __forceinline__ float dpp_mov(float v) {
  return __builtin_bit_cast(float, __builtin_amdgcn_update_dpp(0, __builtin_bit_cast(int, v), CTRL, 0xf, 0xf, true));
}
__device__ __forceinline__ float group_max16(float v) {
  v = fmaxf(v, dpp_mov<0xB1>(v));
  v = fmaxf(v, dpp_mov<0x4E>(v));
  v = fmaxf(v, dpp_mov<0x141>(v));
  v = fmaxf(v, dpp_mov<0x140>(v));
  return v;
}

struct FastDiv { unsigned d, m, s; };
__host__ inline FastDiv make_fastdiv(unsigned d) {
  FastDiv f; f.d = d ? d : 1; f.m = 0; f.s = 0;
  if (f.d == 1) return f;
  unsigned s = 0; while ((1ull << s) < f.d) ++s;
  f.s = s;
  f.m = (unsigned)(((1ull << 32) * ((1ull << s) - f.d)) / f.d + 1ull);
  return f;
// ... 128 lines not shown
```

### marl_amd/csrc/gemm.hip

```cpp
#include <cstdlib>
#include "common.h"
#include "../../include/marl_hip.h"

namespace {

struct LinArgs {
  ConcatSrc x;
  const float* W; long ldw;
  const float* bias;
  float* Y; long ldy;
  int M, N, K;
  int act;
  float beta;
  int groups;
  long gs_x0, gs_x1, gs_w, gs_b, gs_y, gs_m0;
};

template <int AMODE, bool W_KMAJOR, bool BF, bool GATE, int NC>
__global__ __launch_bounds__(256) void linear_kernel(LinArgs a) {
  const int lane = threadIdx.x & 63, wave = threadIdx.x >> 6;
  const int q = lane >> 4, m = lane & 15;
  const int g = blockIdx.z;
  ConcatSrc x = a.x;
  if (x.p0) x.p0 += g * a.gs_x0;
  if (x.p1) x.p1 += g * a.gs_x1;
  if (x.m0) x.m0 += g * a.gs_m0;
  const float* W = a.W + g * a.gs_w;
  const float* bias = a.bias ? a.bias + g * a.gs_b : nullptr;
  float* Y = a.Y + g * a.gs_y;

  const long row0 = (long)blockIdx.x * 128 + wave * 32;
  const int col0 = blockIdx.y * (16 * NC);
  if (row0 >= a.M) return;
  int ct_used = (a.N - col0 + 15) / 16;
  if (ct_used > NC) ct_used = NC;

  long arow[2];
#pragma unroll
  for (int r = 0; r < 2; ++r) {
    long rr = row0 + r * 16 + m;
    arow[r] = rr < a.M ? rr : a.M - 1;
  }
  int bcol[NC];
#pragma unroll
  for (int c = 0; c < NC; ++c) {
    int cc = col0 + c * 16 + m;
    bcol[c] = cc < a.N ? cc : a.N - 1;
  }

  f32x4 acc[2][NC];
#pragma unroll
  for (int r = 0; r < 2; ++r)
#pragma unroll
    for (int c = 0; c < NC; ++c) acc[r][c] = (f32x4){0.f, 0.f, 0.f, 0.f};

  const int K = a.K;
  const int kfast = AMODE ? (x.k0 & ~15) : 0;
  ConcatRow crow[2];
  const float* ap[2];
  const float* mp[2];
  bool aok[2];
#pragma unroll
  for (int r = 0; r < 2; ++r) {
    crow[r] = concat_row(x, arow[r]);
    aok[r] = crow[r].ok0;
    ap[r] = x.p0 + (aok[r] ? crow[r].r0 : 0) * x.ld0 + 4 * q;
    mp[r] = GATE ? x.m0 + (aok[r] ? crow[r].r0 : 0) * x.ldm0 + 4 * q : nullptr;
  }
  const bool wvec = !W_KMAJOR && (a.ldw % 4 == 0) && ((reinterpret_cast<uintptr_t>(W) & 15) == 0);
  auto load = [&](f32x4 (&av)[2], f32x4 (&mv)[2], f32x4 (&bv)[NC], int k0) __attribute__((always_inline)) {
    const int kk = k0 + 4 * q;
#pragma unroll
    for (int r = 0; r < 2; ++r) {
      if (AMODE == 1) av[r] = *reinterpret_cast<const f32x4*>(ap[r] + k0);
      else { av[r][0] = ap[r][k0]; av[r][1] = ap[r][k0 + 1]; av[r][2] = ap[r][k0 + 2]; av[r][3] = ap[r][k0 + 3]; }
      if (GATE) {
        if (AMODE == 1) mv[r] = *reinterpret_cast<const f32x4*>(mp[r] + k0);
        else { mv[r][0] = mp[r][k0]; mv[r][1] = mp[r][k0 + 1]; mv[r][2] = mp[r][k0 + 2]; mv[r][3] = mp[r][k0 + 3]; }
      }
    }
#pragma unroll
    for (int c = 0; c < NC; ++c) {
      if (!W_KMAJOR) {
        const float* wp = W + (long)bcol[c] * a.ldw + kk;
        if (wvec) bv[c] = *reinterpret_cast<const f32x4*>(wp);
        else { bv[c][0] = wp[0]; bv[c][1] = wp[1]; bv[c][2] = wp[2]; bv[c][3] = wp[3]; }
      } else {
#pragma unroll
        for (int i = 0; i < 4; ++i) bv[c][i] = W[(long)(kk + i) * a.ldw + bcol[c]];
      }
    }
  };
  auto mma = [&](const f32x4 (&av)[2], const f32x4 (&mv)[2], const f32x4 (&bv)[NC]) __attribute__((always_inline)) {
    f32x4 am[2];
#pragma unroll
    for (int r = 0; r < 2; ++r) {
      am[r] = aok[r] ? av[r] : (f32x4){0.f, 0.f, 0.f, 0.f};
      if (GATE) {
#pragma unroll
        for (int i = 0; i < 4; ++i) am[r][i] = mv[r][i] > 0.f ? am[r][i] : 0.f;
      }
    }
#pragma unroll
    for (int c = 0; c < NC; ++c) {
      if (c >= ct_used) continue;
#pragma unroll
      for (int r = 0; r < 2; ++r) acc[r][c] = mm16x4<BF>(am[r], bv[c], acc[r][c]);
    }
  };
  if (AMODE && kfast > 0) {
    f32x4 aA[2], bA[NC], aB[2], bB[NC], mA[2], mB[2];
    const int klast = kfast - 16;
    load(aA, mA, bA, 0);
    int k0 = 0;
    while (true) {
      load(aB, mB, bB, k0 + 16 < klast ? k0 + 16 : klast);
      mma(aA, mA, bA);
      k0 += 16;
      if (k0 >= kfast) break;
      load(aA, mA, bA, k0 + 16 < klast ? k0 + 16 : klast);
      mma(aB, mB, bB);
      k0 += 16;
      if (k0 >= kfast) break;
    }
  }
  for (int k0 = kfast; k0 < K; k0 += 16) {
    const int kk = k0 + 4 * q;
    f32x4 av[2], bv[NC];
#pragma unroll
    for (int r = 0; r < 2; ++r)
#pragma unroll
      for (int i = 0; i < 4; ++i) av[r][i] = (kk + i < K) ? concat_at(x, crow[r], kk + i) : 0.f;
#pragma unroll
    for (int c = 0; c < NC; ++c) {
      if (c < ct_used) {
#pragma unroll
        for (int i = 0; i < 4; ++i) {
          float w = 0.f;
          if (kk + i < K) w = W_KMAJOR ? W[(long)(kk + i) * a.ldw + bcol[c]] : W[(long)bcol[c] * a.ldw + kk + i];
          bv[c][i] = w;
        }
      }
    }
#pragma unroll
    for (int c = 0; c < NC; ++c) {
      if (c < ct_used) {
#pragma unroll
        for (int r = 0; r < 2; ++r) acc[r][c] = mm16x4<BF>(av[r], bv[c], acc[r][c]);
      }
    }
  }

#pragma unroll
  for (int c = 0; c < NC; ++c) {
// ... 600 lines not shown
    }
#pragma unroll
    for (int i = 0; i < NX; ++i) {
      const long off = rtab[tb + (xr[i] < 0 ? 0 : xr[i])];
      if (off < 0) zmask |= 1u << i;
      px[i] = *reinterpret_cast<const f32x4*>(a.x.p0 + (off < 0 ? 0 : off) + xc[i]);
    }
  };
  int old_h[2] = {-1, -1}, old_i[2] = {-1, -1};
  if (!cons)
    for (int e = ptid; e < 2 * ti; e += TPT) {
      const int bb = e >= ti ? 1 : 0, ee = e - bb * ti;
      const int r = ee / T4, c = k0 + (ee - r * T4) * 4;
      *reinterpret_cast<f32x4*>(tsm + bb * BUF + TCH * TGP + r * XP + c) = (f32x4){0.f, 0.f, 0.f, 0.f};
    }
  auto stash = [&](const f32x4 (&pg)[NG], const f32x4 (&px)[NX], unsigned zmask, long ch, int b) __attribute__((always_inline)) {
    const int tb = (int)(ch & 7) * TCH;
    float* Gs = tsm + b * BUF;
    float* Xs = Gs + TCH * TGP;
#pragma unroll
    for (int i = 0; i < NG; ++i) {
      const int e = ptid + TPT * i;
      f32x4 v = pg[i];
      if (zmask & (0x100u << i)) v = (f32x4){0.f, 0.f, 0.f, 0.f};
      *reinterpret_cast<f32x4*>(Gs + (e >> 4) * TGP + (e & 15) * 4) = v;
    }
#pragma unroll
    for (int i = 0; i < NX; ++i) {
      if (xr[i] >= 0) {
        f32x4 v = px[i];
        if (zmask & (1u << i)) v = (f32x4){0.f, 0.f, 0.f, 0.f};
        *reinterpret_cast<f32x4*>(Xs + xr[i] * XP + xc[i]) = v;
      }
    }
    if (ptid < TCH && T4 > 0) {
      float* row = Xs + ptid * XP;
      if (old_h[b] >= 0) row[old_h[b]] = 0.f;
      if (old_i[b] >= 0) row[old_i[b]] = 0.f;
      const int hc = htab[tb + ptid], ic = itab[tb + ptid];
      if (hc >= 0) row[hc] = 1.f;
      if (ic >= 0) row[ic] = 1.f;
      old_h[b] = hc; old_i[b] = ic;
    }
  };

  if (wave == 4) {
    resolve_issue(0); resolve_commit(0);
    resolve_issue(2); resolve_commit(2);
  }
  __syncthreads();
  if (!cons) {
    f32x4 gS0[NG], xS0[NX], gS1[NG], xS1[NX];
    unsigned z0 = 0, z1 = 0;
    fetch(gS0, xS0, z0, 0); stash(gS0, xS0, z0, 0, 0);
    fetch(gS0, xS0, z0, 1);
    ST_DECL(2);
    for (long ch = 0; ch < nch; ch += 2) {
      const bool mine = wave == 4 + (int)((ch >> 1) & 3);
      asm volatile("s_waitcnt lgkmcnt(0)\n\ts_barrier" ::: "memory");
      ST_MARK(0);
      if (mine) resolve_issue(ch + 4);
      fetch(gS1, xS1, z1, ch + 2);
      stash(gS0, xS0, z0, ch + 1, 1);
      ST_MARK(1);
      asm volatile("s_waitcnt lgkmcnt(0)\n\ts_barrier" ::: "memory");
      ST_MARK(0);
      fetch(gS0, xS0, z0, ch + 3);
      stash(gS1, xS1, z1, ch + 2, 0);
      if (mine) resolve_commit(ch + 4);
      ST_MARK(1);
    }
    ST_DUMP(2);
    return;
  }

  const int tn = wave & 3;
  f32x4 acc[KTT];
#pragma unroll
  for (int j = 0; j < KTT; ++j) acc[j] = (f32x4){0.f, 0.f, 0.f, 0.f};
  float bs = 0.f;
  ST_DECL(2);
  for (long ch = 0; ch < ((nch + 1) & ~1L); ++ch) {
    asm volatile("s_waitcnt lgkmcnt(0)\n\ts_barrier" ::: "memory");
    ST_MARK(0);
    if (ch >= nch) break;
    const float* Gs = tsm + (int)(ch & 1) * BUF + tn * 16 + m + q * TGP;
    const float* Xs = tsm + (int)(ch & 1) * BUF + TCH * TGP + m + q * XP;
    auto ld = [&](float& gv, float (&xv)[KTT]) __attribute__((always_inline)) {
      gv = Gs[0];
#pragma unroll
      for (int j = 0; j < KTT; ++j) xv[j] = Xs[16 * j];
      Gs += 4 * TGP; Xs += 4 * XP;
    };
    auto mac = [&](float gv, const float (&xv)[KTT]) __attribute__((always_inline)) {
      bs += gv;
#pragma unroll
      for (int j = 0; j < KTT; ++j) acc[j] = mfma16(gv, xv[j], acc[j]);
      __builtin_amdgcn_sched_barrier(0);
    };
    float gA, gB, xA[KTT], xB[KTT];
    ld(gA, xA);
#pragma unroll 1
    for (int st = 0; st < TCH / 4 - 2; st += 2) {
      ld(gB, xB);
      mac(gA, xA);
      ld(gA, xA);
      mac(gB, xB);
    }
    ld(gB, xB);
    mac(gA, xA);
    mac(gB, xB);
    ST_MARK(1);
  }
  ST_DUMP(2);
  const int Kx = K + 1;
  float* slab = a.ws + (long)blockIdx.x * 64 * Kx;
#pragma unroll
  for (int j = 0; j < KTT; ++j) {
    const int k = 16 * j + m;
    if (k < K) {
#pragma unroll
      for (int i = 0; i < 4; ++i) slab[(long)(16 * tn + 4 * q + i) * Kx + k] = acc[j][i];
    }
  }
  bs += __shfl_xor(bs, 16, 64);
  bs += __shfl_xor(bs, 32, 64);
  if (q == 0) slab[(long)(16 * tn + m) * Kx + K] = bs;
}

inline int tall_xp(int K) { const int w = (K + 15) / 16 * 16; return (w % 32 == 16) ? w : w + 16; }
inline int try_wgrad_tall(WgradArgs& a, size_t ws_bytes, hipStream_t s) {
  if (!marl_switches()->wgrad_tall) return -1;
  if (a.N != 64 || a.groups != 1 || a.Yact || !a.gvec || !a.xvec || a.M < 4096 || a.x.k1 || a.x.m0 || !a.x.p0) return -1;
  if (a.x.nhot > 1 || a.x.k0 < 16 || a.x.k0 > 224) return -1;
  if ((a.x.k0 & 3) && (a.x.nhot || a.x.nid || (a.x.ld0 & 3))) return -1;
  const int KT = (a.K + 15) / 16;
  if (KT > 14) return -1;
  const int XP = tall_xp(a.K);
  const size_t lds = (size_t)2 * TCH * (TGP + XP) * sizeof(float) + 8 * TCH * (sizeof(long) + 2 * sizeof(int));
  const bool wide = a.x.k0 > 192;
  if (lds > (wide ? 160 : 80) * 1024) return -1;
  int slabs = a.slabs;
  if (slabs == 256 && ws_bytes >= (size_t)512 * 64 * (a.K + 1) * sizeof(float)) slabs = 512;
  a.slabs = slabs;
  const void* fn = KT <= 6 ? (const void*)wgrad_tall_kernel<6, 3> : KT <= 10 ? (const void*)wgrad_tall_kernel<10, 5>
                   : wide ? (const void*)wgrad_tall_kernel<14, 7> : (const void*)wgrad_tall_kernel<14, 6>;
  hipError_t e = hipFuncSetAttribute(fn, hipFuncAttributeMaxDynamicSharedMemorySize, (int)lds);
  if (e != hipSuccess) return (int)e;
  int xp = XP;
  void* kargs[] = {(void*)&a, (void*)&xp};
  e = hipLaunchKernel(fn, dim3(slabs), dim3(512), kargs, lds, s);
  if (e != hipSuccess) return (int)e;
  return 0;
}

__global__ __launch_bounds__(256) void wgrad_thin_kernel(WgradArgs a) {
  __shared__ float part[256 * 4 + 256];
  const int tid = threadIdx.x;
  const int KG = (a.K + 3) >> 2, RL = 256 / KG;
  const int cg = tid % KG, rl = tid / KG;
  const long per = ((long)a.M + gridDim.x - 1) / gridDim.x;
  const long r_begin = (long)blockIdx.x * per;
  long r_end = r_begin + per; if (r_end > a.M) r_end = a.M;
  f32x4 acc = {0.f, 0.f, 0.f, 0.f};
  float gs = 0.f;
  if (rl < RL) {
    const float* xp = a.x.p0 + 4 * cg;
    long r = r_begin + rl;
    for (; r + 3L * RL < r_end; r += 4L * RL) {
      float g[4]; f32x4 xv[4];
#pragma unroll
      for (int u = 0; u < 4; ++u) { g[u] = a.G[(r + (long)u * RL) * a.ldg]; xv[u] = *reinterpret_cast<const f32x4*>(xp + (r + (long)u * RL) * a.x.ld0); }
#pragma unroll
      for (int u = 0; u < 4; ++u) { acc += g[u] * xv[u]; gs += g[u]; }
    }
    for (; r < r_end; r += RL) {
      const float g = a.G[r * a.ldg];
      acc += g * *reinterpret_cast<const f32x4*>(xp + r * a.x.ld0);
      gs += g;
    }
  }
  *reinterpret_cast<f32x4*>(part + tid * 4) = acc;
  if (cg == 0 && rl < RL) part[1024 + rl] = gs;
  __syncthreads();
  float* slab = a.ws + (long)blockIdx.x * (a.K + 1);
  if (tid < a.K) {
    float t = 0.f;
    for (int j = 0; j < RL; ++j) t += part[(j * KG) * 4 + tid];
    slab[tid] = t;
  } else if (tid == a.K) {
    float t = 0.f;
    for (int j = 0; j < RL; ++j) t += part[1024 + j];
    slab[a.K] = t;
  }
}

inline int try_wgrad_thin(WgradArgs& a, hipStream_t s) {
  if (a.N != 1 || a.groups != 1 || a.Yact || !a.xvec || a.M < 4096 || a.K > 252 || (a.x.ld0 & 3)) return -1;
  if (!a.x.p0 || a.x.k0 != a.K || a.x.k1 || a.x.nhot || a.x.nid || a.x.m0 || a.x.rpe0 || a.x.emap0) return -1;
  if (a.x.ld0 < (a.K + 3) / 4 * 4) return -1;
  hipLaunchKernelGGL(wgrad_thin_kernel, dim3(a.slabs), dim3(256), 0, s, a);
  return 0;
}

struct WredArgs {
  const float* ws; float* dW; long lddw; float* db;
  int N, K, slabs, groups; long gs_dw, gs_db;
};

constexpr int RSG = 16;
__global__ __launch_bounds__(64 * RSG) void wgrad_reduce_kernel(WredArgs a) {
  __shared__ float part[RSG][64];
  const int Kext = a.K + 1;
  const long per = (long)a.N * Kext;
  const long total = per * a.groups;
  const int el = threadIdx.x & 63, sg = threadIdx.x >> 6;
  const long e = (long)blockIdx.x * 64 + el;
  float s = 0.f;
  if (e < total) {
    const int g = (int)(e / per);
    const long r = e - (long)g * per;
    const long stride = (long)a.groups * per;
    const float* p = a.ws + (long)g * per + r;
    int sl = sg;
    for (; sl + 7 * RSG < a.slabs; sl += 8 * RSG) {
      float v[8];
#pragma unroll
      for (int u = 0; u < 8; ++u) v[u] = p[(long)(sl + u * RSG) * stride];
#pragma unroll
      for (int u = 0; u < 8; ++u) s += v[u];
    }
    for (; sl < a.slabs; sl += RSG) s += p[(long)sl * stride];
  }
  part[sg][el] = s;
  __syncthreads();
  if (sg == 0 && e < total) {
    const int g = (int)(e / per);
    const long r = e - (long)g * per;
    const int n = (int)(r / Kext), k = (int)(r - (long)n * Kext);
    float v = part[0][el];
#pragma unroll
    for (int u = 1; u < RSG; ++u) v += part[u][el];
    if (k < a.K) a.dW[g * a.gs_dw + (long)n * a.lddw + k] += v;
    else if (a.db) a.db[g * a.gs_db + n] += v;
  }
}

inline ConcatSrc to_src(const marl_src_t* s) {
  ConcatSrc c;
  c.p0 = s->p0; c.ld0 = s->ld0; c.k0 = s->k0;
  c.p1 = s->p1; c.ld1 = s->ld1; c.k1 = s->k1;
  c.idx = s->idx; c.nhot = s->nhot; c.hot_w = s->hot_w; c.nid = s->nid;
  c.m0 = s->m0; c.ldm0 = s->ldm0;
  c.rpe0 = s->rpe0; c.bs0 = s->bs0; c.off0 = s->off0;
  c.rpei = s->rpei; c.bsi = s->bsi; c.offi = s->offi;
  c.emap0 = s->emap0;
  c.fd0 = make_fastdiv((unsigned)(s->rpe0 > 0 ? s->rpe0 : 1));
  c.fdi = make_fastdiv((unsigned)(s->rpei > 0 ? s->rpei : 1));
  c.fdn = make_fastdiv((unsigned)(s->nid > 0 ? s->nid : 1));
  return c;
}

inline bool aligned16(const void* p) { return (reinterpret_cast<uintptr_t>(p) & 15) == 0; }

}

ST_DEFINE_SETTER(marl_debug_stamps_wgrad)

extern "C" int marl_linear(const marl_src_t* x, const float* W, long ldw, int w_kmajor, const float* bias,
                           float* Y, long ldy, int M, int N, int K, int act, float beta,
                           const marl_group_t* grp, void* stream) {
  if (M <= 0 || N <= 0 || K <= 0) return 0;
  LinArgs a;
  a.x = to_src(x);
  if (concat_width(a.x) != K) return (int)hipErrorInvalidValue;
  a.W = W; a.ldw = ldw; a.bias = bias; a.Y = Y; a.ldy = ldy; a.M = M; a.N = N; a.K = K;
  a.act = act; a.beta = beta;
  a.groups = grp ? grp->groups : 1;
  a.gs_x0 = grp ? grp->gs_x0 : 0; a.gs_x1 = grp ? grp->gs_x1 : 0; a.gs_w = grp ? grp->gs_w : 0;
  a.gs_b = grp ? grp->gs_b : 0; a.gs_y = grp ? grp->gs_y : 0; a.gs_m0 = grp ? grp->gs_m0 : 0;
  int amode = 0;
  const bool gate = a.x.m0 != nullptr;
  if (a.x.p0 && a.x.k0 >= 16) {
    bool al = (a.x.ld0 % 4 == 0) && aligned16(a.x.p0) && (a.gs_x0 % 4 == 0);
    if (gate) al = al && (a.x.ldm0 % 4 == 0) && aligned16(a.x.m0) && (a.gs_m0 % 4 == 0);
    amode = al ? 1 : 2;
  }
  const bool bf = (act & 0x100) != 0;
  const int nc = (!bf && N > 64 && N <= 80) ? 5 : 4;
  dim3 grid((M + 127) / 128, (N + 16 * nc - 1) / (16 * nc), a.groups), block(256);
  hipStream_t s = (hipStream_t)stream;
  a.act = act & 0xff;
#define LIN_GT(AM, KM, BFV, NCV) do { if (gate) hipLaunchKernelGGL((linear_kernel<AM, KM, BFV, true, NCV>), grid, block, 0, s, a); \
                                     else hipLaunchKernelGGL((linear_kernel<AM, KM, BFV, false, NCV>), grid, block, 0, s, a); } while (0)
#define LIN_KM(AM, BFV, NCV) do { if (w_kmajor) LIN_GT(AM, true, BFV, NCV); else LIN_GT(AM, false, BFV, NCV); } while (0)
#define LIN_AM(BFV, NCV) do { if (amode == 1) LIN_KM(1, BFV, NCV); else if (amode == 2) LIN_KM(2, BFV, NCV); else LIN_KM(0, BFV, NCV); } while (0)
  if (bf) LIN_AM(true, 4);
  else if (nc == 5) LIN_AM(false, 5);
  else LIN_AM(false, 4);
#undef LIN_AM
#undef LIN_KM
#undef LIN_GT
  MARL_CHECK_LAUNCH();
  return 0;
}

extern "C" size_t marl_linear_wgrad_workspace(int M, int N, int K, int groups) {
  int slabs = marl_wgrad_slabs(M);
  if (groups == 1 && ((N <= 80 && K + 1 <= 80) || N == 64)) slabs *= 2;
  return (size_t)slabs * groups * N * (K + 4) * sizeof(float);
}

extern "C" int marl_wgrad_slabs(int M) {
  long chunks = ((long)M + 63) / 64;
  long s = chunks / 8;
  if (s < 1) s = 1;
  if (s > 256) s = 256;
  return (int)s;
}

extern "C" int marl_linear_wgrad(const float* G, long ldg, const float* Yact, long ldya, const marl_src_t* x,
                                 float* dW, long lddw, float* db, int M, int N, int K, int flags,
                                 const marl_group_t* grp, float* ws, size_t ws_bytes, void* stream) {
  if (M <= 0 || N <= 0 || K <= 0) return 0;
  const int groups = grp ? grp->groups : 1;
  if (ws_bytes < marl_linear_wgrad_workspace(M, N, K, groups)) return (int)hipErrorInvalidValue;
  WgradArgs a;
  a.G = G; a.ldg = ldg; a.Yact = Yact; a.ldya = ldya; a.x = to_src(x);
  if (concat_width(a.x) != K) return (int)hipErrorInvalidValue;
  a.ws = ws; a.M = M; a.N = N; a.K = K; a.slabs = marl_wgrad_slabs(M);
  a.nyb = (N + 63) / 64; a.groups = groups;
  a.gs_g = grp ? grp->gs_y : 0; a.gs_ya = grp ? grp->gs_m0 : 0;
  a.gs_x0 = grp ? grp->gs_x0 : 0; a.gs_x1 = grp ? grp->gs_x1 : 0;
  a.gvec = (ldg % 4 == 0) && aligned16(G) && (a.gs_g % 4 == 0) &&
           (!Yact || ((ldya % 4 == 0) && aligned16(Yact) && (a.gs_ya % 4 == 0)));
  a.xvec = a.x.p0 && !a.x.m0 && (a.x.ld0 % 4 == 0) && aligned16(a.x.p0) && (a.gs_x0 % 4 == 0);
  hipStream_t s = (hipStream_t)stream;
  const bool bf = (flags & 1) != 0;
  if (!bf) {
    const int slabs0 = a.slabs;
    const int rc = try_wgrad_tall(a, ws_bytes, s);
    if (rc > 0) return rc;
    if (rc == 0) {
      MARL_CHECK_LAUNCH();
      WredArgs r;
      r.ws = ws; r.dW = dW; r.lddw = lddw; r.db = db; r.N = N; r.K = K; r.slabs = a.slabs; r.groups = 1; r.gs_dw = 0; r.gs_db = 0;
      const long total = (long)N * (K + 1);
      hipLaunchKernelGGL(wgrad_reduce_kernel, dim3((unsigned)((total + 63) / 64)), dim3(64 * RSG), 0, s, r);
      MARL_CHECK_LAUNCH();
      return 0;
    }
    a.slabs = slabs0;
  }
  if (!bf && a.N == 64 && groups == 1 && !Yact && a.gvec && a.xvec && a.M >= 4096 && !a.x.k1 && !a.x.m0 && a.x.k0 >= 64 &&
      K - 64 > 64) {
    const int c_rest = a.x.k0 >= 128 ? 128 : 64;
    if ((K - c_rest + 15) / 16 <= 5) {
      size_t ws_off = 0;
      int c0 = 0;
      for (int pass = 0; c0 < K; ++pass) {
        WgradArgs b = a;
        const bool perm = c0 < c_rest;
        const int kw = perm ? 64 : K - c0;
        b.x.p0 = a.x.p0 + c0;
        b.x.k0 = perm ? 64 : a.x.k0 - c0;
        if (perm) { b.x.idx = nullptr; b.x.nhot = 0; b.x.hot_w = 0; b.x.nid = 0; }
        b.K = kw;
        b.ws = ws + ws_off;
        if (try_wgrad_direct(b, s) != 0) return (int)hipErrorInvalidValue;
        MARL_CHECK_LAUNCH();
        WredArgs r;
        r.ws = b.ws; r.dW = dW + c0; r.lddw = lddw; r.db = pass == 0 ? db : nullptr; r.N = N; r.K = kw; r.slabs = a.slabs;
        r.groups = 1; r.gs_dw = 0; r.gs_db = 0;
        const long total = (long)N * (kw + 1);
        hipLaunchKernelGGL(wgrad_reduce_kernel, dim3((unsigned)((total + 63) / 64)), dim3(64 * RSG), 0, s, r);
        MARL_CHECK_LAUNCH();
        ws_off += (size_t)a.slabs * N * (kw + 1);
        c0 += kw;
      }
      return 0;
    }
  }
  int done = try_wgrad_thin(a, s);
  if (done != 0) done = bf ? -1 : try_wgrad_direct(a, s);
  bool one_base = a.x.p0 && !a.x.m0 && !a.x.nid && a.x.k0 < 16384 && a.x.k1 < 16384 && a.x.nhot < 16384 && a.x.hot_w < 0xfff0;
  for (int c4 = 0; one_base && c4 < K; c4 += 4) {
    auto seg = [&](int k) { return k < a.x.k0 ? 0 : (k - a.x.k0 < a.x.k1 ? 1 : 2); };
    const int kl = c4 + 3 < K ? c4 + 3 : K - 1;
    if (seg(c4) != seg(kl)) one_base = false;
  }
  if (done != 0 && !bf && groups == 1 && N <= WF && K + 1 <= WF && a.gvec && ldg >= (N + 3) / 4 * 4 &&
      (!Yact || ldya >= (N + 3) / 4 * 4) && M >= 2048 && one_base) {
    const size_t lds = (size_t)2 * WCH * WFS * sizeof(float) + (size_t)2 * WCH * 4 * sizeof(long) + (size_t)5 * 256 * 16;
    const long chunks = ((long)M + WCH - 1) / WCH;
    a.slabs = (int)(2L * a.slabs < chunks ? 2L * a.slabs : (chunks < 1 ? 1 : chunks));
    const void* fn = Yact ? (const void*)wgrad_full_kernel<true> : (const void*)wgrad_full_kernel<false>;
    hipError_t e = hipFuncSetAttribute(fn, hipFuncAttributeMaxDynamicSharedMemorySize, (int)lds);
    if (e != hipSuccess) return (int)e;
    if (Yact) hipLaunchKernelGGL(wgrad_full_kernel<true>, dim3(a.slabs), dim3(256), lds, s, a);
    else hipLaunchKernelGGL(wgrad_full_kernel<false>, dim3(a.slabs), dim3(256), lds, s, a);
    done = 0;
  }
  if (done != 0) {
    dim3 grid(a.slabs, a.nyb * groups, (K + 1 + 63) / 64), block(256);
    if (bf) hipLaunchKernelGGL(wgrad_kernel<true>, grid, block, 0, s, a);
    else hipLaunchKernelGGL(wgrad_kernel<false>, grid, block, 0, s, a);
  }
  MARL_CHECK_LAUNCH();
  WredArgs r;
  r.ws = ws; r.dW = dW; r.lddw = lddw; r.db = db; r.N = N; r.K = K; r.slabs = a.slabs; r.groups = groups;
  r.gs_dw = grp ? grp->gs_w : 0; r.gs_db = grp ? grp->gs_b : 0;
  long total = (long)N * (K + 1) * groups;
  hipLaunchKernelGGL(wgrad_reduce_kernel, dim3((unsigned)((total + 63) / 64)), dim3(64 * RSG), 0, s, r);
  MARL_CHECK_LAUNCH();
  return 0;
}
```

### marl_amd/csrc/optim.hip

```cpp
#include "common.h"
#include <string.h>
#include "../../include/marl_hip.h"

namespace {
constexpr int TPB = 256;
constexpr int MAXB = 1024;

__global__ void sumsq_kernel(const float* g, long n, float* ws) {
  __shared__ float sh[TPB / 64];
  float s = 0.f;
  for (long i = (long)blockIdx.x * TPB + threadIdx.x; i < n; i += (long)gridDim.x * TPB) s += g[i] * g[i];
  s = wave_sum(s);
  if ((threadIdx.x & 63) == 0) sh[threadIdx.x >> 6] = s;
  __syncthreads();
  if (threadIdx.x == 0) ws[blockIdx.x] = sh[0] + sh[1] + sh[2] + sh[3];
}

__global__ void sumsq_finish_kernel(const float* ws, int nb, float* out) {
  __shared__ float sh[TPB];
  float s = 0.f;
  for (int b = threadIdx.x; b < nb; b += TPB) s += ws[b];
  sh[threadIdx.x] = s;
  __syncthreads();
  for (int o = TPB / 2; o > 0; o >>= 1) {
    if (threadIdx.x < o) sh[threadIdx.x] += sh[threadIdx.x + o];
    __syncthreads();
  }
  if (threadIdx.x == 0) out[0] = sh[0];
}

__device__ __forceinline__ float grad_scale(const float* sumsq, const float* den, float clip) {
  const float inv = den ? 1.f / den[0] : 1.f;
  const float norm = sqrtf(sumsq[0]) * inv;
  float coef = clip / (norm + 1e-6f);
  coef = coef < 1.f ? coef : 1.f;
  return inv * coef;
}

__global__ void rmsprop_kernel(float* p, const float* g, float* sq, long n, float lr, float alpha, float eps,
                               float clip, const float* sumsq, const float* den) {
  const float sc = grad_scale(sumsq, den, clip);
  for (long i = (long)blockIdx.x * TPB + threadIdx.x; i < n; i += (long)gridDim.x * TPB) {
    const float gi = g[i] * sc;
    const float s = alpha * sq[i] + (1.f - alpha) * gi * gi;
    sq[i] = s;
    p[i] -= lr * gi / (sqrtf(s) + eps);
  }
}

__global__ void adam_kernel(float* p, const float* g, float* m, float* v, long n, float lr, float b1, float b2,
                            float eps, float bc1, float bc2s, float clip, const float* sumsq, const float* den) {
  const float sc = grad_scale(sumsq, den, clip);
  for (long i = (long)blockIdx.x * TPB + threadIdx.x; i < n; i += (long)gridDim.x * TPB) {
    const float gi = g[i] * sc;
    const float mi = b1 * m[i] + (1.f - b1) * gi;
    const float vi = b2 * v[i] + (1.f - b2) * gi * gi;
    m[i] = mi; v[i] = vi;
    p[i] -= (lr / bc1) * mi / (sqrtf(vi) / bc2s + eps);
  }
}

inline int blocks_for(long n) {
  long b = (n + TPB - 1) / TPB;
  if (b > MAXB) b = MAXB;
  if (b < 1) b = 1;
  return (int)b;
}
}

extern "C" size_t marl_sumsq_workspace(long n) { return MAXB * sizeof(float); }

extern "C" int marl_grad_sumsq(const float* g, long n, float* sumsq, float* ws, void* stream) {
  const int nb = blocks_for(n);
  hipLaunchKernelGGL(sumsq_kernel, dim3(nb), dim3(TPB), 0, (hipStream_t)stream, g, n, ws);
  MARL_CHECK_LAUNCH();
  hipLaunchKernelGGL(sumsq_finish_kernel, dim3(1), dim3(TPB), 0, (hipStream_t)stream, (const float*)ws, nb, sumsq);
  MARL_CHECK_LAUNCH();
  return 0;
}

extern "C" int marl_rmsprop_step(float* p, const float* g, float* sq, long n, float lr, float alpha, float eps,
                                 float clip, const float* sumsq, const float* den, void* stream) {
  if (n <= 0) return 0;
  hipLaunchKernelGGL(rmsprop_kernel, dim3(blocks_for(n)), dim3(TPB), 0, (hipStream_t)stream, p, g, sq, n, lr, alpha,
                     eps, clip, sumsq, den);
  MARL_CHECK_LAUNCH();
  return 0;
}

extern "C" int marl_adam_step(float* p, const float* g, float* m, float* v, long n, float lr, float beta1,
                              float beta2, float eps, float bc1, float bc2_sqrt, float clip, const float* sumsq,
                              const float* den, void* stream) {
  if (n <= 0) return 0;
  hipLaunchKernelGGL(adam_kernel, dim3(blocks_for(n)), dim3(TPB), 0, (hipStream_t)stream, p, g, m, v, n, lr, beta1,
                     beta2, eps, bc1, bc2_sqrt, clip, sumsq, den);
  MARL_CHECK_LAUNCH();
  return 0;
}

static MarlSwitches g_switches = {1, 1, 4, 1, 1, 0, 1};
extern "C" const MarlSwitches* marl_switches(void) { return &g_switches; }
static int* switch_slot(const char* name) {
  if (!name) return nullptr;
  struct { const char* n; int* p; } tab[] = {{"fwd_xs", &g_switches.fwd_xs}, {"fwd_w2l", &g_switches.fwd_w2l},
                                             {"bwd_pipe_max_rt", &g_switches.bwd_pipe_max_rt}, {"wgrad_tall", &g_switches.wgrad_tall},
                                             {"wide_res", &g_switches.wide_res}, {"rollout_v1", &g_switches.rollout_v1}, {"unroll_r6", &g_switches.unroll_r6}};
  for (auto& t : tab)
    if (!strcmp(t.n, name)) return t.p;
  return nullptr;
}
extern "C" int marl_experiment_set(const char* name, int value) {
  int* p = switch_slot(name);
  if (!p) return -1;
  *p = value;
  return 0;
}
extern "C" int marl_experiment_get(const char* name) {
  int* p = switch_slot(name);
  return p ? *p : (-2147483647 - 1);
}

#ifndef MARL_SRC_HASH
#define MARL_SRC_HASH "unknown"
#endif
extern "C" const char* marl_hip_version(void) { return "marl_hip 0.4 (gfx950) src " MARL_SRC_HASH; }
```

### marl_amd/experiments.py

```python
from __future__ import annotations

import contextlib
import os
import warnings

LIB_DEFAULTS = {"fwd_xs": 1, "fwd_w2l": 1, "bwd_pipe_max_rt": 4, "wgrad_tall": 1, "wide_res": 1, "rollout_v1": 0, "unroll_r6": 1}
HOST_DEFAULTS = {"no_pair": 0, "no_chain": 0, "chain_split": None, "mlp3_keep": 1, "x6_bwd_min_wg": 1, "force_reducer": 0}


def _env_int(name, default):
    v = os.environ.get("MARL_" + name.upper())
    if v is None or v == "":
        return default
    try:
        return int(v)
    except ValueError:
        warnings.warn("MARL_%s=%r ignored (want an integer)" % (name.upper(), v))
        return default


_lib_values = {k: _env_int(k, d) for k, d in LIB_DEFAULTS.items()}
_host_values = {k: _env_int(k, d) for k, d in HOST_DEFAULTS.items()}
if _host_values["chain_split"] is not None and not (_host_values["chain_split"] == 0 or
                                                      (8 <= _host_values["chain_split"] <= 248 and _host_values["chain_split"] % 8 == 0)):
    warnings.warn("MARL_CHAIN_SPLIT=%r ignored (want 0 or a multiple of 8 in 8..248)" % _host_values["chain_split"])
    _host_values["chain_split"] = None
_applied = None
generation = 0


def apply(lib):
    global _applied
    _applied = lib
    for k, v in _lib_values.items():
        if v != LIB_DEFAULTS[k]:
            rc = lib.marl_experiment_set(k.encode(), int(v))
            assert rc == 0, "marl_experiment_set(%s) failed" % k


def get(name):
    if name in _host_values:
        return _host_values[name]
    if name in _lib_values:
        if _applied is not None:
            _lib_values[name] = int(_applied.marl_experiment_get(name.encode()))
        return _lib_values[name]
    raise KeyError(name)


def set(name, value):
    global generation
    generation += 1
    if name in _host_values:
        _host_values[name] = value
        return
    if name not in _lib_values:
        raise KeyError(name)
    _lib_values[name] = int(value)
    from . import _lib
    rc = _lib.load().marl_experiment_set(name.encode(), int(value))
    assert rc == 0, name


@contextlib.contextmanager
def override(**kw):
    old = {k: get(k) for k in kw}
    try:
        for k, v in kw.items():
            set(k, v)
        yield
    finally:
        for k, v in old.items():
            set(k, v)
```

### marl_amd/ops.py

```python
from __future__ import annotations

import ctypes as C

import torch

from . import _lib
from ._lib import (MarlSrc, MarlGroup, MarlAgentWeights, MarlAgentGrads, MarlQmixWeights, MarlMlp3Weights,
                   MarlQtranWeights, MarlRtwWeights, MarlWorldWeights, MarlWorldGrads, MarlMaicWeights, MarlMaicGrads, MarlMaicInfer,
                   MarlMaicInferGrads, check)


def _p(t):
    return None if t is None else C.c_void_p(t.data_ptr())


def _stream():
    return C.c_void_p(torch.cuda.current_stream().cuda_stream)


def _f32(t):
    assert t.dtype == torch.float32 and t.is_cuda, "expected a CUDA float32 tensor"
    return t


def _i32(t):
    assert t.dtype == torch.int32 and t.is_cuda, "expected a CUDA int32 tensor"
    return t


class Workspace:

    def __init__(self):
        self.bufs = {}
        self.gen = 0

    def get(self, name, nbytes, device):
        n = (int(nbytes) + 3) // 4
        b = self.bufs.get(name)
        if b is None or b.numel() < n or b.device != device:
            b = torch.empty(max(n, 1), dtype=torch.float32, device=device)
            self.bufs[name] = b
            self.gen += 1
        return b

    def snapshot(self):
        return list(self.bufs.values())


WS = Workspace()


class Rows:

    def __init__(self, t, remap, emap=None):
        self.t, self.remap, self.emap = t, remap, emap
        self.device = t.device


def src(x0=None, x1=None, idx=None, nhot=0, hot_w=0, nid=0, gate=None, remap0=None, remapi=None, k0=None, emap0=None):
    s = MarlSrc()
    keep = []
    if isinstance(x0, Rows):
        x0, remap0, emap0 = x0.t, x0.remap, x0.emap
    if x0 is not None:
        _f32(x0); assert x0.dim() == 2 and x0.stride(1) == 1
        s.p0, s.ld0, s.k0 = x0.data_ptr(), x0.stride(0), (x0.shape[1] if k0 is None else k0)
        keep.append(x0)
    if x1 is not None:
        _f32(x1); assert x1.dim() == 2 and x1.stride(1) == 1
        s.p1, s.ld1, s.k1 = x1.data_ptr(), x1.stride(0), x1.shape[1]
        keep.append(x1)
    if idx is not None:
        _i32(idx)
        s.idx, s.nhot, s.hot_w = idx.data_ptr(), nhot, hot_w
        keep.append(idx)
    s.nid = nid
    if gate is not None:
        _f32(gate); assert gate.dim() == 2 and gate.stride(1) == 1
        s.m0, s.ldm0 = gate.data_ptr(), gate.stride(0)
        keep.append(gate)
    if remap0 is not None:
        s.rpe0, s.bs0, s.off0 = remap0
    if emap0 is not None:
        assert remap0 is not None and emap0.dtype == torch.int32 and emap0.is_contiguous()
        s.emap0 = emap0.data_ptr()
        keep.append(emap0)
    if remapi is not None:
        s.rpei, s.bsi, s.offi = remapi
    s._keep = keep
    return s


def src_width(s):
    return s.k0 + s.k1 + s.nhot * s.hot_w + s.nid


def group(groups, x0=0, x1=0, w=0, b=0, y=0, m0=0):
    return MarlGroup(groups, x0, x1, w, b, y, m0)


def linear(x, W, bias, Y, M, N, K, act=0, beta=0.0, w_kmajor=False, ldw=None, grp=None, bf16=False):
    lib = _lib.load()
    if bf16:
        act |= 0x100
    if ldw is None:
        ldw = W.stride(0) if W.dim() == 2 else (N if w_kmajor else K)
    ldy = Y.stride(0) if Y.dim() == 2 else N
    assert src_width(x) == K, (src_width(x), K)
    check(lib.marl_linear(C.byref(x), _p(_f32(W)), ldw, 1 if w_kmajor else 0, _p(bias), _p(_f32(Y)), ldy,
                          M, N, K, act, float(beta), C.byref(grp) if grp is not None else None, _stream()),
          "marl_linear")


def linear_wgrad(dY, x, dW, db, M, N, K, Yact=None, grp=None, lddw=None, bf16=False):
    lib = _lib.load()
    flags = 1 if bf16 else 0
    g = grp.groups if grp is not None else 1
    nbytes = lib.marl_linear_wgrad_workspace(M, N, K, g)
    ws = WS.get("wgrad", nbytes, dY.device)
    if lddw is None:
        lddw = dW.stride(0) if dW.dim() == 2 else K
    assert src_width(x) == K, (src_width(x), K)
    check(lib.marl_linear_wgrad(_p(_f32(dY)), dY.stride(0) if dY.dim() == 2 else N,
                                _p(Yact), (Yact.stride(0) if Yact.dim() == 2 else N) if Yact is not None else 0,
                                C.byref(x), _p(_f32(dW)), lddw, _p(db), M, N, K, flags,
                                C.byref(grp) if grp is not None else None, _p(ws), ws.numel() * 4, _stream()),
          "marl_linear_wgrad")


def agent_weights(params):
    w = MarlAgentWeights()
    w.fc1_w, w.fc1_b = params["fc1.weight"].data_ptr(), params["fc1.bias"].data_ptr()
    w.w_ih, w.w_hh = params["rnn.weight_ih"].data_ptr(), params["rnn.weight_hh"].data_ptr()
    w.b_ih, w.b_hh = params["rnn.bias_ih"].data_ptr(), params["rnn.bias_hh"].data_ptr()
    w.fc2_w, w.fc2_b = params["fc2.weight"].data_ptr(), params["fc2.bias"].data_ptr()
    w.H = params["rnn.weight_hh"].shape[1]
    for k in ("fc1.weight", "rnn.weight_ih", "rnn.weight_hh", "fc2.weight"):
        assert params[k].is_contiguous() and params[k].dtype == torch.float32 and params[k].is_cuda
    w._keep = params
    return w


def agent_unroll_fwd(w, obs, obs_bs, obs_t0, ufed, u_bs, u_t0, h0, q, hs, h_last, saved,
                     B, T, N, O, A, last_action=True, reuse_network=True, ep_len=None, ep_map=None, cu_budget=0, gi_out=None,
                     gi_in=None):
    lib = _lib.load()
    check(lib.marl_agent_unroll_fwd(C.byref(w), _p(_f32(obs)), obs_bs, obs_t0, _p(ufed), u_bs, u_t0, _p(ep_len),
                                    _p(_i32(ep_map)) if ep_map is not None else None, _p(h0),
                                    _p(_f32(q)), _p(hs), _p(h_last), _p(saved), B, T, N, O, A,
                                    1 if last_action else 0, 1 if reuse_network else 0, int(cu_budget),
                                    _p(_f32(gi_out)) if gi_out is not None else None,
                                    _p(_f32(gi_in)) if gi_in is not None else None, _stream()),
          "marl_agent_unroll_fwd")


def agent_unroll_x6_supported(B, T, N, O, A, last_action=True, reuse_network=True):
    return bool(_lib.load().marl_agent_unroll_x6_supported(B, T, N, O, A, 1 if last_action else 0, 1 if reuse_network else 0))


def agent_unroll_x6_plain_r6(B, T, N, O, A, last_action=True, reuse_network=True, cu_budget=0):
    return bool(_lib.load().marl_agent_unroll_x6_plain_r6(B, T, N, O, A, 1 if last_action else 0, 1 if reuse_network else 0, int(cu_budget)))


def agent_unroll_fwd_x6(w, obs, obs_bs, obs_t0, ufed, u_bs, u_t0, h0, q, hs, h_last, saved, B, T, N, O, A, last_action=True,
                        reuse_network=True, ep_len=None, ep_map=None, cu_budget=0, gi_out=None, gi_in=None):
    if saved is None and gi_in is None and hs is None and agent_unroll_x6_plain_r6(B, T, N, O, A, last_action, reuse_network, cu_budget):
        assert obs.numel() < 2 ** 30 and (ufed is None or ufed.numel() < 2 ** 30), "observation storage beyond 4 GB: set MARL_UNROLL_R6=0"
    check(_lib.load().marl_agent_unroll_fwd_x6(C.byref(w), _p(_f32(obs)), obs_bs, obs_t0, _p(ufed), u_bs, u_t0, _p(ep_len),
                                               _p(_i32(ep_map)) if ep_map is not None else None, _p(h0), _p(_f32(q)), _p(hs),
                                               _p(h_last), _p(saved), B, T, N, O, A, 1 if last_action else 0,
                                               1 if reuse_network else 0, int(cu_budget),
                                               _p(_f32(gi_out)) if gi_out is not None else None,
                                               _p(_f32(gi_in)) if gi_in is not None else None, _stream()),
          "marl_agent_unroll_fwd_x6")


UNROLL_FAMILIES = ("f32-pipe", "f32-multi", "x6", "x6-r6")
UNROLL_INPUT_PATHS = ("element", "vector", "half", "w2l")


def agent_unroll_fwd_plan(x6, B, T, N, O, A, last_action=True, reuse_network=True, cu_budget=0, saved=False, gi_out=False,
                          gi_in=False, hs=True, obs_aligned=True, h_aligned=True):
    flags = (1 if saved else 0) | (2 if gi_out else 0) | (4 if gi_in else 0) | (8 if hs else 0) | (16 if obs_aligned else 0) | (32 if h_aligned else 0)
    plan = (C.c_int * 8)()
    if _lib.load().marl_agent_unroll_fwd_plan(1 if x6 else 0, B, T, N, O, A, 1 if last_action else 0, 1 if reuse_network else 0,
                                              int(cu_budget), flags, plan) != 0:
        return None
    return tuple(plan)


def saved_shape(T, B, N, planes=6, H=64):
    return (T + (1 if planes == 6 else 0), (B * N + 15) // 16 * 16, planes, H)


def saved_plane(saved, plane, rows):
    T, R16, P, H = saved.shape
    t = saved.reshape(T, R16 // 16, P, 4, 4, 16, 4)[:, :, plane]
    return t.permute(0, 1, 3, 5, 2, 4).reshape(T, R16, H)[:, :rows]


def agent_unroll_reuse_supported(B, T, N, O, A, cu_budget=0):
    return bool(_lib.load().marl_agent_unroll_reuse_supported(B, T, N, O, A, int(cu_budget)))


def agent_unroll_bwd_x6_supported(B, T, N, A, sparse_dq=True):
    return bool(_lib.load().marl_agent_unroll_bwd_x6_supported(B, T, N, A, 1 if sparse_dq else 0))


def agent_unroll_bwd(w, dq, dhs, saved, hs, dxp, dh0, grads, B, T, N, A, dq_idx=None, dq_val=None, dq_idx2=None,
                     dq_val2=None, dq_gdiv=1, x6=False):
    lib = _lib.load()
    g = MarlAgentGrads()
    g.w_ih, g.w_hh = grads["rnn.weight_ih"].data_ptr(), grads["rnn.weight_hh"].data_ptr()
    g.b_ih, g.b_hh = grads["rnn.bias_ih"].data_ptr(), grads["rnn.bias_hh"].data_ptr()
    g.fc2_w, g.fc2_b = grads["fc2.weight"].data_ptr(), grads["fc2.bias"].data_ptr()
    for v in grads.values():
        assert v.is_contiguous() and v.dtype == torch.float32 and v.is_cuda
    if x6:
        assert dq is None and dq_idx is not None and dq_val is not None and dq_idx.is_contiguous() and dq_val.is_contiguous()
        _i32(dq_idx); _f32(dq_val)
        if dq_idx2 is not None:
            assert dq_val2 is not None and dq_idx2.is_contiguous() and dq_val2.is_contiguous()
            _i32(dq_idx2); _f32(dq_val2)
        ws = WS.get("agent_bwd_x6", lib.marl_agent_bwd_x6_workspace(B, N, A), saved.device)
        check(lib.marl_agent_unroll_bwd_x6(C.byref(w), _p(dq_idx), _p(dq_val), _p(dq_idx2), _p(dq_val2), int(dq_gdiv), _p(dhs),
                                           _p(_f32(saved)), _p(_f32(dxp)), _p(dh0), C.byref(g), _p(ws), ws.numel() * 4, B, T, N, A,
                                           _stream()), "marl_agent_unroll_bwd_x6")
        return
    ws = WS.get("agent_bwd", lib.marl_agent_bwd_workspace(B, N, A), saved.device)
    if dq_idx is not None:
        assert dq is None and dq_val is not None and dq_idx.is_contiguous() and dq_val.is_contiguous()
        _i32(dq_idx); _f32(dq_val)
    if dq_idx2 is not None:
        assert dq_idx is not None and dq_val2 is not None and dq_idx2.is_contiguous() and dq_val2.is_contiguous()
        _i32(dq_idx2); _f32(dq_val2)
    check(lib.marl_agent_unroll_bwd(C.byref(w), _p(_f32(dq)) if dq is not None else None, _p(dq_idx), _p(dq_val),
                                    _p(dq_idx2), _p(dq_val2), int(dq_gdiv), _p(dhs),
                                    _p(_f32(saved)), _p(hs), _p(_f32(dxp)),
                                    _p(dh0), C.byref(g), _p(ws), ws.numel() * 4, B, T, N, A, _stream()),
          "marl_agent_unroll_bwd")


def q_gather(q, idx, out, rows, A, avail=None, mask_val=0.0):
    check(_lib.load().marl_q_gather(_p(_f32(q)), _p(_i32(idx)), _p(avail), float(mask_val), _p(_f32(out)), rows, A,
                                    _stream()), "marl_q_gather")


def q_masked_max(q, avail, mask_val, out_max, out_arg, rows, A):
    check(_lib.load().marl_q_masked_max(_p(_f32(q)), _p(avail), float(mask_val), _p(out_max), _p(out_arg), rows, A,
                                        _stream()), "marl_q_masked_max")


def q_double_select(q_sel, q_val, avail, mask_val, out_val, out_arg, rows, A):
    check(_lib.load().marl_q_double_select(_p(_f32(q_sel)), _p(_f32(q_val)), _p(avail), float(mask_val), _p(_f32(out_val)),
                                           _p(out_arg), rows, A, _stream()), "marl_q_double_select")


def q_scatter(dq, idx1, g1, idx2, g2, rows, A, gdiv=1):
    check(_lib.load().marl_q_scatter(_p(_f32(dq)), _p(idx1), _p(g1), _p(idx2), _p(g2), rows, A, gdiv, _stream()),
          "marl_q_scatter")


def vec_add(a, b, out, n):
    check(_lib.load().marl_vec_add(_p(_f32(a)), _p(_f32(b)), _p(_f32(out)), n, _stream()), "marl_vec_add")


def _ld(t, D):
    return t.stride(0) if (t.dim() == 2 and t.shape[1] == D and t.stride(1) == 1) else D


def agent_sum(inp, out, rows, N, D):
    check(_lib.load().marl_agent_sum(_p(_f32(inp)), _ld(inp, D), _p(_f32(out)), _ld(out, D), rows, N, D, _stream()),
          "marl_agent_sum")


def agent_bcast(inp, out, rows, N, D, accumulate=False):
    check(_lib.load().marl_agent_bcast(_p(_f32(inp)), _ld(inp, D), _p(_f32(out)), _ld(out, D), rows, N, D,
                                       1 if accumulate else 0, _stream()), "marl_agent_bcast")


def qmix_mix_fwd(hy, b2, q, q_tot, rows, N, E, w22=None, b22=None):
    check(_lib.load().marl_qmix_mix_fwd(_p(_f32(hy)), hy.stride(0), _p(b2), _p(w22), _p(b22), _p(_f32(q)), _p(_f32(q_tot)), rows,
                                        N, E, _stream()), "marl_qmix_mix_fwd")


def qmix_mix_bwd(hy, q, dq_tot, dhy, db2, dq, rows, N, E, w22=None):
    assert dhy.stride(0) == hy.stride(0)
    check(_lib.load().marl_qmix_mix_bwd(_p(_f32(hy)), hy.stride(0), _p(_f32(q)), _p(_f32(dq_tot)), _p(w22), _p(_f32(dhy)),
                                        _p(_f32(db2)), _p(_f32(dq)), rows, N, E, _stream()), "marl_qmix_mix_bwd")


def qmix_tail_supported(S, E, s):
    return E == 32 and qtran_state_parts_supported(S, s)


def qmix_tail_fwd(s, rows, S, b1_w, b1_b, h_w, h_b, hy, c_b1, c_h):
    assert b1_w.stride(1) == 1 and h_w.stride(1) == 1 and b1_w.stride(0) == h_w.stride(0) and hy.stride(1) == 1
    x = src(s)
    check(_lib.load().marl_qmix_tail_fwd(C.byref(x), rows, S, _p(_f32(b1_w)), b1_w.stride(0), _p(_f32(b1_b)), _p(_f32(h_w)),
                                         h_w.stride(0), _p(_f32(h_b)), _p(_f32(hy)), hy.stride(0), c_b1, c_h, _stream()),
          "marl_qmix_tail_fwd")


def qplex_mix_fwd(w_raw, v, q, max_q, key, ag, ac, v_tot, a_tot, lam_out, rows, N, K, weighted, minus_one):
    check(_lib.load().marl_qplex_mix_fwd(_p(w_raw), _p(v), _p(q), _p(max_q), _p(key), _p(ag), _p(ac), _p(v_tot),
                                         _p(a_tot), _p(lam_out), rows, N, K, int(weighted), int(minus_one), _stream()),
          "marl_qplex_mix_fwd")


def qplex_mix_bwd(w_raw, q, max_q, key, ag, ac, g, dq, dw_raw, dv, dkey, dag, dac, rows, N, K, weighted, minus_one):
    check(_lib.load().marl_qplex_mix_bwd(_p(w_raw), _p(q), _p(max_q), _p(key), _p(ag), _p(ac), _p(g), _p(dq),
                                         _p(dw_raw), _p(dv), _p(dkey), _p(dag), _p(dac), rows, N, K, int(weighted),
                                         int(minus_one), _stream()), "marl_qplex_mix_bwd")


_FT_OUT = {}


def replay_gather(idx, src, out):
    assert idx.dtype == torch.int64 and idx.is_cuda and idx.is_contiguous()
    B, T, N, A = int(idx.numel()), src.T, src.N, src.A
    for t in (src.u, src.r, src.term, src.padded, src.length, src.won, src.avail, out.u, out.u_act, out.r, out.term, out.padded,
              out.length, out.won, out.avail_next, out.o_map):
        assert t.is_cuda and t.is_contiguous()
    assert src.u.dtype == torch.int32 and src.length.dtype == torch.int32 and src.won.dtype == torch.int32
    check(_lib.load().marl_replay_gather(_p(idx), B, T, N, A, _p(src.u), _p(_f32(src.r)), _p(_f32(src.term)), _p(_f32(src.padded)),
                                         _p(src.length), _p(src.won), _p(_f32(src.avail)), _p(_i32(out.o_map)), _p(_i32(out.u)),
                                         _p(_i32(out.u_act)), _p(_f32(out.r)), _p(_f32(out.term)), _p(_f32(out.padded)),
                                         _p(_i32(out.length)), _p(_i32(out.won)), _p(_f32(out.avail_next)),
                                         _p(getattr(out, "avail_cur", None)), _stream()),
          "marl_replay_gather")


def first_terminated_len(term, T):
    t2 = term.reshape(term.shape[0], -1)
    assert t2.dtype == torch.float32 and t2.is_cuda and t2.stride(1) == 1
    ring = _FT_OUT.get(t2.device)
    if ring is None:
        ring = _FT_OUT[t2.device] = [torch.zeros(8, dtype=torch.int32, device=t2.device), 0]
    out = ring[0][ring[1] % 8:ring[1] % 8 + 1]
    ring[1] += 1
    check(_lib.load().marl_first_terminated_len(_p(t2), t2.stride(0), t2.shape[0], min(T, t2.shape[1]), _p(out), _stream()),
          "marl_first_terminated_len")
    return out


def td_loss(q_tot, q_tgt, r, term, padded, gamma, dq_tot, out2, rows):
    lib = _lib.load()
    ws = WS.get("loss", lib.marl_loss_workspace(rows), q_tot.device)
    check(lib.marl_td_loss(_p(_f32(q_tot)), _p(_f32(q_tgt)), _p(_f32(r)), _p(_f32(term)), _p(_f32(padded)),
                           float(gamma), _p(_f32(dq_tot)), _p(_f32(out2)), _p(ws), rows, _stream()), "marl_td_loss")


def qtran_loss(jq, jq_tgt, v, jq_hat, qs_opt, qs_nopt, r, term, padded, gamma, lam_opt, lam_nopt,
               d_jq, d_v, d_qso, d_qsn, out4, rows):
    lib = _lib.load()
    ws = WS.get("loss", lib.marl_loss_workspace(rows), jq.device)
    check(lib.marl_qtran_loss(_p(jq), _p(jq_tgt), _p(v), _p(jq_hat), _p(qs_opt), _p(qs_nopt), _p(r), _p(term),
                              _p(padded), float(gamma), float(lam_opt), float(lam_nopt), _p(d_jq), _p(d_v), _p(d_qso),
                              _p(d_qsn), _p(out4), _p(ws), rows, _stream()), "marl_qtran_loss")


def td_lambda_returns(q_next_tot, r, term, padded, gamma, lam, out, B, T):
    lib = _lib.load()
    for t in (q_next_tot, r, term, padded, out):
        assert _f32(t).is_contiguous() and t.numel() >= B * T, "td_lambda_returns: contiguous (B, T) float32 arrays"
    check(lib.marl_td_lambda_returns(_p(q_next_tot), _p(r), _p(term), _p(padded), float(gamma), float(lam), _p(out),
                                     int(B), int(T), _stream()), "marl_td_lambda_returns")
    return out


def policy_probs(logits, avail, eps, pi, rows, A):
    for t in (logits, avail, pi):
        assert _f32(t).is_contiguous() and t.numel() >= rows * A
    check(_lib.load().marl_policy_probs(_p(logits), _p(avail), float(eps), _p(pi), rows, A, _stream()), "marl_policy_probs")
    return pi


def policy_loss_bwd(logits, avail, u, G, v, padded, eps, dlogits, logp, out2, rows, N, A):
    lib = _lib.load()
    for t, n in ((logits, rows * A), (avail, rows * A), (dlogits, rows * A), (logp, rows), (G, rows // N), (v, rows // N),
# ... 567 lines not shown
```

Before: 73.53 million.

## Emit tiled dxp from x6 BPTT and consume it in a new x6 fc1 wgrad kernel

The x6 backward kernel can now write the fc1 pre-activation gradient in an MFMA-tile layout with vectorized f32x4 stores instead of scattered per-row scalar stores. A new tall wgrad kernel reads that tiled gradient directly and splits the gathered inputs into bf16x6 planes to compute the fc1 weight gradient, with a producer/consumer wave split and LDS staging. This is meant to remove the strided row scatter and to speed up the fc1 wgrad GEMM. In exchange it adds a padded tile buffer with a spare tile and extra masking for partial tiles, and it applies only when H is 64 and dhs is absent.

```diff
diff --git a/include/marl_hip.h b/include/marl_hip.h
--- a/include/marl_hip.h
+++ b/include/marl_hip.h
@@ -37,6 +37,9 @@
                       const marl_group_t* grp, float* ws, size_t ws_bytes, void* stream);
 size_t marl_linear_wgrad_workspace(int M, int N, int K, int groups);
 int marl_wgrad_slabs(int M);
+int marl_linear_wgrad_x6t_supported(const marl_src_t* x, int B, int T, int N, int K);
+int marl_linear_wgrad_x6t(const float* g_tiled, const marl_src_t* x, float* dW, long lddw, float* db, int B, int T, int N, int K,
+                          float* ws, size_t ws_bytes, void* stream);
 
 int marl_agent_unroll_fwd(const marl_agent_weights_t* w, const float* obs, long obs_bs, int obs_t0,
                           const int* ufed, long u_bs, int u_t0, const int* ep_len, const int* ep_map,
@@ -170,6 +173,11 @@
 int marl_agent_unroll_bwd_x6(const marl_agent_weights_t* w, const int* dq_idx, const float* dq_val, const int* dq_idx2,
                              const float* dq_val2, int dq_gdiv, const float* dhs, const float* saved, float* dxp, float* dh0,
                              const marl_agent_grads_t* g, float* ws, size_t ws_bytes, int B, int T, int N, int A, void* stream);
+size_t marl_agent_bwd_x6_dxp_tiled_bytes(int B, int T, int N);
+int marl_agent_unroll_bwd_x6_tiled(const marl_agent_weights_t* w, const int* dq_idx, const float* dq_val, const int* dq_idx2,
+                                   const float* dq_val2, int dq_gdiv, const float* dhs, const float* saved, float* dxp,
+                                   float* dxp_tiled, float* dh0, const marl_agent_grads_t* g, float* ws, size_t ws_bytes, int B,
+                                   int T, int N, int A, void* stream);
 
 int marl_mlp3_x6_supported(const marl_src_t* x, int K1, int H1, int H2, int N3, int groups);
 int marl_mlp3_x6_fwd_save(const marl_mlp3_weights_t* w, const marl_src_t* x, float* Y, long ldy, long gs_y,
diff --git a/marl_amd/_lib.py b/marl_amd/_lib.py
--- a/marl_amd/_lib.py
+++ b/marl_amd/_lib.py
@@ -98,6 +98,8 @@
     "marl_linear": (I, [SRC, P, L, I, P, P, L, I, I, I, I, F, GRP, P]),
     "marl_linear_wgrad": (I, [P, L, P, L, SRC, P, L, P, I, I, I, I, GRP, P, SZ, P]),
     "marl_linear_wgrad_workspace": (SZ, [I, I, I, I]),
+    "marl_linear_wgrad_x6t_supported": (I, [SRC, I, I, I, I]),
+    "marl_linear_wgrad_x6t": (I, [P, SRC, P, L, P, I, I, I, I, P, SZ, P]),
     "marl_wgrad_slabs": (I, [I]),
     "marl_agent_unroll_fwd": (I, [AW, P, L, I, P, L, I, P, P, P, P, P, P, P, I, I, I, I, I, I, I, I, P, P, P]),
     "marl_agent_unroll_reuse_supported": (I, [I, I, I, I, I, I]),
@@ -109,6 +111,8 @@
     "marl_agent_unroll_bwd_x6_supported": (I, [I, I, I, I, I]),
     "marl_agent_bwd_x6_workspace": (SZ, [I, I, I]),
     "marl_agent_unroll_bwd_x6": (I, [AW, P, P, P, P, I, P, P, P, P, AG, P, SZ, I, I, I, I, P]),
+    "marl_agent_unroll_bwd_x6_tiled": (I, [AW, P, P, P, P, I, P, P, P, P, P, AG, P, SZ, I, I, I, I, P]),
+    "marl_agent_bwd_x6_dxp_tiled_bytes": (SZ, [I, I, I]),
     "marl_agent_unroll_bwd": (I, [AW, P, P, P, P, P, I, P, P, P, P, P, AG, P, SZ, I, I, I, I, P]),
     "marl_replay_gather": (I, [P, I, I, I, I] + [P] * 17 + [P]),
     "marl_q_gather": (I, [P, P, P, F, P, L, I, P]),
diff --git a/marl_amd/algorithm/common.py b/marl_amd/algorithm/common.py
--- a/marl_amd/algorithm/common.py
+++ b/marl_amd/algorithm/common.py
@@ -310,7 +310,6 @@
     H = args.rnn_hidden_dim
     M = B * T * N
     dev = saved.device
-    dxp = buf.get("dxp", (B, T, N, H), dev)
     w = mac.agent.weights()
     ag = mac.agent
     grads = {"rnn.weight_ih": ag.rnn.weight_ih.grad, "rnn.weight_hh": ag.rnn.weight_hh.grad,
@@ -318,8 +317,6 @@
              "fc2.weight": ag.fc2.weight.grad, "fc2.bias": ag.fc2.bias.grad}
     x6 = (x6_mode(args) and dq is None and dq_idx is not None
           and (B * N + 31) // 32 >= experiments.get("x6_bwd_min_wg") and ops.agent_unroll_bwd_x6_supported(B, T, N, A))
-    ops.agent_unroll_bwd(w, dq, dhs, saved, hs, dxp, None, grads, B, T, N, A, dq_idx=dq_idx, dq_val=dq_val,
-                         dq_idx2=dq_idx2, dq_val2=dq_val2, dq_gdiv=dq_gdiv, x6=x6)
     obs, obs_bs, obs_t0 = db.o_cur if which == "cur" else db.o_next
     remap0 = None if (obs_bs == T * N and obs_t0 == 0) else (T * N, obs_bs, obs_t0 * N)
     kw = {}
@@ -330,6 +327,15 @@
         remap0 = (T * N, obs_bs, obs_t0 * N)
     xin = ops.src(obs.reshape(-1, O), nid=N if args.reuse_network else 0, remap0=remap0, emap0=emap, **kw)
     I = O + (A if args.last_action else 0) + (N if args.reuse_network else 0)
+    if x6 and dhs is None and H == 64 and ops.linear_wgrad_x6t_supported(xin, B, T, N, I):
+        dxt = buf.get("dxp_tiled", (ops.dxp_tiled_numel(B, T, N),), dev)
+        ops.agent_unroll_bwd(w, dq, dhs, saved, hs, None, None, grads, B, T, N, A, dq_idx=dq_idx, dq_val=dq_val,
+                             dq_idx2=dq_idx2, dq_val2=dq_val2, dq_gdiv=dq_gdiv, x6=x6, dxp_tiled=dxt)
+        ops.linear_wgrad(None, xin, ag.fc1.weight.grad, ag.fc1.bias.grad, M, H, I, bf16=False, g_tiled=dxt, btn=(B, T, N))
+        return
+    dxp = buf.get("dxp", (B, T, N, H), dev)
+    ops.agent_unroll_bwd(w, dq, dhs, saved, hs, dxp, None, grads, B, T, N, A, dq_idx=dq_idx, dq_val=dq_val,
+                         dq_idx2=dq_idx2, dq_val2=dq_val2, dq_gdiv=dq_gdiv, x6=x6)
     ops.linear_wgrad(dxp.view(M, H), xin, ag.fc1.weight.grad, ag.fc1.bias.grad, M, H, I, bf16=False)
 
 
diff --git a/marl_amd/csrc/agent_bwd_x6.hip b/marl_amd/csrc/agent_bwd_x6.hip
--- a/marl_amd/csrc/agent_bwd_x6.hip
+++ b/marl_amd/csrc/agent_bwd_x6.hip
@@ -21,6 +21,8 @@
   const float* dhs;
   const float* saved;
   float* dxp;
+  float* dxt;
+  unsigned spare_tile;
   float* dh0;
   float* ws;
   int B, T, N, A;
@@ -115,7 +117,7 @@
 __device__ __forceinline__ F3 splitn(const f32x4 (&x)[2]) { return split8(x[0], x[1]); }
 __device__ __forceinline__ F3h splitn(const f32x4 (&x)[1]) { return split4(x[0]); }
 
-template <bool DHS, bool TWO, int NT>
+template <bool DHS, bool TWO, int NT, bool TILED = false>
 __global__ __launch_bounds__(BNT, 2) void agent_bwd_x6_kernel(BX6Args a) {
   typedef typename FW<NT>::T FWT;
   extern __shared__ __attribute__((aligned(16))) char smem[];
@@ -287,10 +289,18 @@
         }
         __builtin_amdgcn_sched_barrier(0);
         const f32x4 dx = da + db;
-#pragma unroll
-        for (int r = 0; r < 4; ++r) {
-          const int ri = rowidx[16 * tt + 4 * q + r];
-          if (ri >= 0) a.dxp[(unsigned)(ri + t * a.N) * (unsigned)H + (unsigned)u] = (xmask >> (4 * tt + r)) & 1u ? dx[r] : 0.f;
+        if (TILED) {
+          f32x4 o;
+#pragma unroll
+          for (int r = 0; r < 4; ++r) o[r] = (xmask >> (4 * tt + r)) & 1u ? dx[r] : 0.f;
+          const unsigned tix = (tt == 1 && tl[1] == tl[0]) ? a.spare_tile : (unsigned)t * (unsigned)NTILES + (unsigned)tl[tt];
+          *reinterpret_cast<f32x4*>(a.dxt + ((size_t)tix * 1024u + (unsigned)s * 256u) + lane * 4) = o;
+        } else {
+#pragma unroll
+          for (int r = 0; r < 4; ++r) {
+            const int ri = rowidx[16 * tt + 4 * q + r];
+            if (ri >= 0) a.dxp[(unsigned)(ri + t * a.N) * (unsigned)H + (unsigned)u] = (xmask >> (4 * tt + r)) & 1u ? dx[r] : 0.f;
+          }
         }
       }
       __builtin_amdgcn_sched_barrier(0);
@@ -346,6 +356,14 @@
       for (int tt = 0; tt < NT; ++tt)
 #pragma unroll
         for (int r = 0; r < 4; ++r) mk |= xn[tt][r] > 0.f ? 1u << (4 * tt + r) : 0u;
+      if (TILED) {
+#pragma unroll
+        for (int tt = 0; tt < NT; ++tt) {
+          const long left = a.R - 16 * tl[tt] - 4 * q;
+          const unsigned ok = left >= 4 ? 0xfu : left <= 0 ? 0u : (1u << (int)left) - 1u;
+          mk &= ~(0xfu << (4 * tt)) | (ok << (4 * tt));
+        }
+      }
       XM[(t & 1) * 256 + s * 64 + lane] = mk;
     };
     auto dw2 = [&](const int4* qt, const FWT& hb) {
@@ -505,19 +523,38 @@
   return (size_t)(n2 + n1) * slab_floats(A) * sizeof(float);
 }
 
+extern "C" size_t marl_agent_bwd_x6_dxp_tiled_bytes(int B, int T, int N) {
+  if (B < 1 || T < 1 || N < 1) return 0;
+  const double tiles = (double)(((long)B * N + 15) / 16) * T + 1.0;
+  if (tiles * 4096.0 >= 4294967296.0) return 0;
+  return (size_t)tiles * 4096;
+}
+
 extern "C" int marl_agent_unroll_bwd_x6(const marl_agent_weights_t* w, const int* dq_idx, const float* dq_val, const int* dq_idx2,
                                         const float* dq_val2, int dq_gdiv, const float* dhs, const float* saved, float* dxp,
                                         float* dh0, const marl_agent_grads_t* g, float* ws, size_t ws_bytes, int B, int T, int N,
                                         int A, void* stream) {
+  return marl_agent_unroll_bwd_x6_tiled(w, dq_idx, dq_val, dq_idx2, dq_val2, dq_gdiv, dhs, saved, dxp, nullptr, dh0, g, ws, ws_bytes,
+                                        B, T, N, A, stream);
+}
+
+extern "C" int marl_agent_unroll_bwd_x6_tiled(const marl_agent_weights_t* w, const int* dq_idx, const float* dq_val, const int* dq_idx2,
+                                              const float* dq_val2, int dq_gdiv, const float* dhs, const float* saved, float* dxp,
+                                              float* dxp_tiled, float* dh0, const marl_agent_grads_t* g, float* ws, size_t ws_bytes,
+                                              int B, int T, int N, int A, void* stream) {
   if (B <= 0 || T <= 0) return 0;
+  if (dxp_tiled && (dhs || !marl_agent_bwd_x6_dxp_tiled_bytes(B, T, N) || (reinterpret_cast<uintptr_t>(dxp_tiled) & 15)))
+    return (int)hipErrorInvalidValue;
+  if (!dxp_tiled && !dxp) return (int)hipErrorInvalidValue;
   if (w->H != H || !marl_agent_unroll_bwd_x6_supported(B, T, N, A, dq_idx != nullptr) || !dq_val || (dq_idx2 && !dq_val2))
     return (int)hipErrorInvalidValue;
   if (ws_bytes < marl_agent_bwd_x6_workspace(B, N, A) || (reinterpret_cast<uintptr_t>(saved) & 15)) return (int)hipErrorInvalidValue;
   BX6Args a;
   a.Wih = w->w_ih; a.Whh = w->w_hh; a.W2 = w->fc2_w;
   a.dq_idx = dq_idx; a.dq_val = dq_val; a.dq_idx2 = dq_idx2; a.dq_val2 = dq_val2; a.dq_gdiv = dq_gdiv > 1 ? dq_gdiv : 1;
-  a.dhs = dhs; a.saved = saved; a.dxp = dxp; a.dh0 = dh0; a.ws = ws;
+  a.dhs = dhs; a.saved = saved; a.dxp = dxp; a.dxt = dxp_tiled; a.dh0 = dh0; a.ws = ws;
   a.B = B; a.T = T; a.N = N; a.A = A; a.R = (long)B * N;
+  a.spare_tile = (unsigned)(((a.R + 15) >> 4) * T);
   long n2, n1;
   bx6_plan(a.R, n2, n1);
   const size_t lds = (size_t)GBUF + 8 * FRB + 32 * H * 4 + 3 * 32 * 16 + 2 * 32 * 4 + 2 * 256 * 4 + 4 * 256 * 4;
@@ -528,6 +565,9 @@
     const long nwg = pass == 0 ? n2 : n1;
     if (nwg == 0) continue;
     const void* fn = pass == 0 ? BX6_PICK(2) : BX6_PICK(1);
+    if (dxp_tiled)
+      fn = pass == 0 ? (dq_idx2 ? (const void*)agent_bwd_x6_kernel<false, true, 2, true> : (const void*)agent_bwd_x6_kernel<false, false, 2, true>)
+                     : (dq_idx2 ? (const void*)agent_bwd_x6_kernel<false, true, 1, true> : (const void*)agent_bwd_x6_kernel<false, false, 1, true>);
     a.tile_base = pass == 0 ? 0 : 2 * n2;
     a.slab_base = pass == 0 ? 0 : (int)n2;
     hipError_t e = hipFuncSetAttribute(fn, hipFuncAttributeMaxDynamicSharedMemorySize, (int)lds);
diff --git a/marl_amd/csrc/common.h b/marl_amd/csrc/common.h
--- a/marl_amd/csrc/common.h
+++ b/marl_amd/csrc/common.h
@@ -7,7 +7,7 @@
 #define WG_BARRIER() asm volatile("s_waitcnt lgkmcnt(0)\n\ts_barrier" ::: "memory")
 
 struct MarlSwitches {
-  int fwd_xs, fwd_w2l, bwd_pipe_max_rt, wgrad_tall, wide_res, rollout_v1, unroll_r6;
+  int fwd_xs, fwd_w2l, bwd_pipe_max_rt, wgrad_tall, wide_res, rollout_v1, unroll_r6, fc1_x6;
 };
 extern "C" const MarlSwitches* marl_switches(void);
 
diff --git a/marl_amd/csrc/gemm.hip b/marl_amd/csrc/gemm.hip
--- a/marl_amd/csrc/gemm.hip
+++ b/marl_amd/csrc/gemm.hip
@@ -1,5 +1,5 @@
 #include <cstdlib>
-#include "common.h"
+#include "x6.h"
 #include "../../include/marl_hip.h"
 
 namespace {
@@ -906,6 +906,217 @@
   e = hipLaunchKernel(fn, dim3(slabs), dim3(512), kargs, lds, s);
   if (e != hipSuccess) return (int)e;
   return 0;
+}
+
+struct TallX6Args {
+  ConcatSrc x;
+  const float* gt;
+  float* ws;
+  int K, T, Nag;
+  unsigned NP, NTILES, R;
+  unsigned nchunks;
+  FastDiv fN, fNP;
+};
+
+template <int KTT, int NX>
+__global__ __launch_bounds__(512, KTT >= 14 ? 2 : 4) void wgrad_tall_kernel_x6(TallX6Args a) {
+  extern __shared__ __attribute__((aligned(16))) char xsm[];
+  typedef __attribute__((address_space(3))) s16x4 lds_s16x4;
+  const int tid = threadIdx.x, lane = tid & 63, wave = __builtin_amdgcn_readfirstlane(tid >> 6);
+  const bool cons = wave < 4;
+  const int ptid = tid - 256;
+  constexpr int XP = (KTT + 1) * 16;
+  constexpr int PLB = TCH * XP * 2, BUFB = 3 * PLB;
+  const int K = a.K, k0 = a.x.k0;
+  long* rtab = reinterpret_cast<long*>(xsm + 2 * BUFB);
+  int* htab = reinterpret_cast<int*>(rtab + 8 * TCH);
+  int* itab = htab + 8 * TCH;
+  const unsigned per = (a.nchunks + gridDim.x - 1) / gridDim.x;
+  const unsigned c_begin = blockIdx.x * per;
+  const unsigned c_end = c_begin + per < a.nchunks ? c_begin + per : a.nchunks;
+  const long nch = c_end > c_begin ? (long)(c_end - c_begin) : 0;
+  const int D4 = k0 >> 2;
+  const int di = TCH * D4;
+
+  for (int e = tid; e < 2 * BUFB / 16; e += 512) reinterpret_cast<i32x4*>(xsm)[e] = (i32x4){0, 0, 0, 0};
+
+  int rs_em = 0, rs_u = -1, rs_w = 0, rs_n = -1;
+  bool rs_ok0 = false, rs_oki = false, rs_live = false;
+  auto resolve_issue = [&](long ch) {
+    const unsigned cg = c_begin + (unsigned)ch + (unsigned)(lane >> 5);
+    rs_live = cg < c_end;
+    const unsigned cgc = rs_live ? cg : 0u;
+    const unsigned t = fastdiv(cgc, a.fNP), pr = cgc - t * a.NP;
+    unsigned rho = 32u * pr + (unsigned)(lane & 31);
+    if (rho >= a.R) { rs_live = false; rho = 0; }
+    const unsigned bb = fastdiv(rho, a.fN), n = rho - bb * (unsigned)a.Nag;
+    const unsigned ur = (bb * (unsigned)a.T + t) * (unsigned)a.Nag + n;
+    const long row = (long)ur;
+    unsigned e = ur; long w = 0;
+    rs_ok0 = true;
+    if (a.x.rpe0) { e = fastdiv(ur, a.x.fd0); w = (long)(ur - e * (unsigned)a.x.rpe0) + a.x.off0; rs_ok0 = w >= 0; }
+    rs_w = (int)w;
+    rs_em = (a.x.emap0 && a.x.rpe0) ? a.x.emap0[e] : (int)e;
+    long ri = row; rs_oki = true;
+    if (a.x.rpei) { const unsigned ei = fastdiv(ur, a.x.fdi); const long wi = (long)(ur - ei * (unsigned)a.x.rpei) + a.x.offi;
+                    rs_oki = wi >= 0; ri = (long)ei * a.x.bsi + wi; }
+    rs_u = (a.x.nhot && rs_oki) ? a.x.idx[ri * a.x.nhot] : -1;
+    rs_n = a.x.nid ? (int)(ur - fastdiv(ur, a.x.fdn) * (unsigned)a.x.nid) : -1;
+  };
+  auto resolve_commit = [&](long ch) {
+    const int b = (int)(ch & 7) * TCH + lane;
+    const long r0 = a.x.rpe0 ? (long)rs_em * a.x.bs0 + rs_w : (long)rs_em;
+    rtab[b] = (rs_ok0 && rs_live) ? r0 * a.x.ld0 : -1;
+    htab[b] = (rs_live && rs_u >= 0 && rs_u < a.x.hot_w) ? k0 + rs_u : -1;
+    itab[b] = (rs_live && rs_n >= 0) ? k0 + a.x.nhot * a.x.hot_w + rs_n : -1;
+  };
+
+  int xr[NX], xc[NX];
+#pragma unroll
+  for (int i = 0; i < NX; ++i) {
+    const int e = ptid + TPT * i;
+    xr[i] = -1; xc[i] = 0;
+    if (ptid >= 0 && e < di) { const int r = e / D4; xr[i] = r; xc[i] = (e - r * D4) * 4; }
+  }
+  auto fetch = [&](f32x4 (&px)[NX], unsigned& zmask, long ch) __attribute__((always_inline)) {
+    const int tb = (int)(ch & 7) * TCH;
+    zmask = 0;
+#pragma unroll
+    for (int i = 0; i < NX; ++i) {
+      const long off = rtab[tb + (xr[i] < 0 ? 0 : xr[i])];
+      if (off < 0) zmask |= 1u << i;
+      px[i] = *reinterpret_cast<const f32x4*>(a.x.p0 + (off < 0 ? 0 : off) + xc[i]);
+    }
+  };
+  int old_h[2] = {-1, -1}, old_i[2] = {-1, -1};
+  auto stash = [&](const f32x4 (&px)[NX], unsigned zmask, long ch, int b) __attribute__((always_inline)) {
+    const int tb = (int)(ch & 7) * TCH;
+    char* Xs = xsm + b * BUFB;
+#pragma unroll
+    for (int i = 0; i < NX; ++i) {
+      if (xr[i] >= 0) {
+        f32x4 v = px[i];
+        if (zmask & (1u << i)) v = (f32x4){0.f, 0.f, 0.f, 0.f};
+        const F3h f = split4(v);
+        char* p = Xs + (xr[i] * XP + xc[i]) * 2;
+        *reinterpret_cast<i32x2*>(p) = f.h;
+        *reinterpret_cast<i32x2*>(p + PLB) = f.m;
+        *reinterpret_cast<i32x2*>(p + 2 * PLB) = f.l;
+      }
+    }
+    if (ptid < TCH) {
+      short* row = reinterpret_cast<short*>(Xs) + ptid * XP;
+      if (old_h[b] >= 0) row[old_h[b]] = 0;
+      if (old_i[b] >= 0) row[old_i[b]] = 0;
+      const int hc = htab[tb + ptid], ic = itab[tb + ptid];
+      if (hc >= 0) row[hc] = (short)0x3f80;
+      if (ic >= 0) row[ic] = (short)0x3f80;
+      old_h[b] = hc; old_i[b] = ic;
+    }
+  };
+
+  if (wave == 4) {
+    resolve_issue(0); resolve_commit(0);
+    resolve_issue(2); resolve_commit(2);
+  }
+  __syncthreads();
+  if (!cons) {
+    f32x4 xS0[NX], xS1[NX];
+    unsigned z0 = 0, z1 = 0;
+    fetch(xS0, z0, 0); stash(xS0, z0, 0, 0);
+    fetch(xS0, z0, 1);
+    for (long ch = 0; ch < nch; ch += 2) {
+      const bool mine = wave == 4 + (int)((ch >> 1) & 3);
+      asm volatile("s_waitcnt lgkmcnt(0)\n\ts_barrier" ::: "memory");
+      if (mine) resolve_issue(ch + 4);
+      fetch(xS1, z1, ch + 2);
+      stash(xS0, z0, ch + 1, 1);
+      asm volatile("s_waitcnt lgkmcnt(0)\n\ts_barrier" ::: "memory");
+      fetch(xS0, z0, ch + 3);
+      stash(xS1, z1, ch + 2, 0);
+      if (mine) resolve_commit(ch + 4);
+    }
+    return;
+  }
+
+  const int tn = wave & 3;
+  f32x4 acc[KTT];
+#pragma unroll
+  for (int j = 0; j < KTT; ++j) acc[j] = (f32x4){0.f, 0.f, 0.f, 0.f};
+  float bs = 0.f;
+  const int tb = (((lane >> 4) * 4 + ((lane & 15) >> 2)) * XP + 4 * (lane & 3)) * 2;
+  unsigned lt = fastdiv(c_begin < a.nchunks ? c_begin : 0u, a.fNP);
+  unsigned lp = (c_begin < a.nchunks ? c_begin : 0u) - lt * a.NP;
+  long nload = 0;
+  const float* gbase = a.gt + tn * 256 + lane * 4;
+  auto gload = [&](f32x4& g0, f32x4& g1, unsigned& dead) __attribute__((always_inline)) {
+    const bool live = nload < nch;
+    const unsigned t = live ? lt : 0u, tile0 = live ? 2u * lp : 0u;
+    const bool has1 = tile0 + 1u < a.NTILES;
+    const float* p = gbase + (size_t)(t * a.NTILES + tile0) * 1024u;
+    g0 = *reinterpret_cast<const f32x4*>(p);
+    g1 = *reinterpret_cast<const f32x4*>(has1 ? p + 1024 : p);
+    dead = (live ? 0u : 1u) | ((live && has1) ? 0u : 2u);
+    ++nload;
+    if (++lp == a.NP) { lp = 0; ++lt; }
+  };
+  auto xfrag = [&](const char* p) __attribute__((always_inline)) {
+    F3 f;
+#pragma unroll
+    for (int pl = 0; pl < 3; ++pl) {
+      const s16x4 lo = __builtin_amdgcn_ds_read_tr16_b64_v4i16((lds_s16x4*)(p + pl * PLB));
+      const s16x4 hi = __builtin_amdgcn_ds_read_tr16_b64_v4i16((lds_s16x4*)(p + pl * PLB + 16 * XP * 2));
+      const i32x4 v = __builtin_bit_cast(i32x4, (s16x8)__builtin_shufflevector(lo, hi, 0, 1, 2, 3, 4, 5, 6, 7));
+      if (pl == 0) f.h = v; else if (pl == 1) f.m = v; else f.l = v;
+    }
+    return f;
+  };
+  auto mac = [&](int b, f32x4 g0, f32x4 g1, unsigned dead) __attribute__((always_inline)) {
+    if (dead & 1u) g0 = (f32x4){0.f, 0.f, 0.f, 0.f};
+    if (dead & 2u) g1 = (f32x4){0.f, 0.f, 0.f, 0.f};
+    bs += ((g0[0] + g0[1]) + (g0[2] + g0[3])) + ((g1[0] + g1[1]) + (g1[2] + g1[3]));
+    const F3 A = split8(g0, g1);
+    const char* xb = xsm + b * BUFB + tb;
+#pragma unroll
+    for (int j = 0; j < KTT; j += 2) {
+      const F3 b0 = xfrag(xb + 32 * j), b1 = xfrag(xb + 32 * (j + 1));
+#define OP(p_, q_) acc[j] = mm(A.p_, b0.q_, acc[j]); acc[j + 1] = mm(A.p_, b1.q_, acc[j + 1]);
+      X6_TERMS(OP)
+#undef OP
+    }
+  };
+  f32x4 gA0, gA1, gB0, gB1;
+  unsigned dA, dB;
+  gload(gA0, gA1, dA);
+  gload(gB0, gB1, dB);
+  for (long ch = 0; ch < nch; ch += 2) {
+    asm volatile("s_waitcnt lgkmcnt(0)\n\ts_barrier" ::: "memory");
+    {
+      const f32x4 u0 = gA0, u1 = gA1; const unsigned d = dA;
+      gload(gA0, gA1, dA);
+      mac(0, u0, u1, d);
+    }
+    asm volatile("s_waitcnt lgkmcnt(0)\n\ts_barrier" ::: "memory");
+    {
+      const f32x4 u0 = gB0, u1 = gB1; const unsigned d = dB;
+      gload(gB0, gB1, dB);
+      mac(1, u0, u1, d);
+    }
+  }
+  const int q = lane >> 4, m = lane & 15;
+  const int Kx = K + 1;
+  float* slab = a.ws + (long)blockIdx.x * 64 * Kx;
+#pragma unroll
+  for (int j = 0; j < KTT; ++j) {
+    const int k = 16 * j + m;
+    if (k < K) {
+#pragma unroll
+      for (int i = 0; i < 4; ++i) slab[(long)(16 * tn + 4 * q + i) * Kx + k] = acc[j][i];
+    }
+  }
+  bs += __shfl_xor(bs, 16, 64);
+  bs += __shfl_xor(bs, 32, 64);
+  if (q == 0) slab[(long)(16 * tn + m) * Kx + K] = bs;
 }
 
 __global__ __launch_bounds__(256) void wgrad_thin_kernel(WgradArgs a) {
@@ -1169,3 +1380,53 @@
   MARL_CHECK_LAUNCH();
   return 0;
 }
+
+static bool wgrad_x6t_covers(const ConcatSrc& c, int B, int T, int N, int K) {
+  if (B < 1 || T < 1 || N < 1 || K < 1) return false;
+  const double M = (double)B * T * N;
+  if (M < 4096.0 || M >= 2147483648.0) return false;
+  if (concat_width(c) != K || (K + 15) / 16 > 14) return false;
+  if (!c.p0 || c.m0 || c.k1 || c.nhot > 1 || c.k0 < 16 || c.k0 > 224 || (c.k0 & 3) || (c.ld0 & 3) || !aligned16(c.p0)) return false;
+  return marl_agent_bwd_x6_dxp_tiled_bytes(B, T, N) != 0;
+}
+
+extern "C" int marl_linear_wgrad_x6t_supported(const marl_src_t* x, int B, int T, int N, int K) {
+  if (!x || !marl_switches()->fc1_x6) return 0;
+  return wgrad_x6t_covers(to_src(x), B, T, N, K) ? 1 : 0;
+}
+
+extern "C" int marl_linear_wgrad_x6t(const float* g_tiled, const marl_src_t* x, float* dW, long lddw, float* db, int B, int T, int N,
+                                     int K, float* ws, size_t ws_bytes, void* stream) {
+  if (!g_tiled || !x || !dW || !ws || !aligned16(g_tiled)) return (int)hipErrorInvalidValue;
+  TallX6Args a;
+  a.x = to_src(x);
+  if (!wgrad_x6t_covers(a.x, B, T, N, K)) return (int)hipErrorInvalidValue;
+  const int M = B * T * N;
+  if (ws_bytes < marl_linear_wgrad_workspace(M, 64, K, 1)) return (int)hipErrorInvalidValue;
+  a.gt = g_tiled; a.ws = ws; a.K = K; a.T = T; a.Nag = N;
+  a.R = (unsigned)((long)B * N);
+  a.NTILES = (a.R + 15u) >> 4;
+  a.NP = (a.NTILES + 1u) >> 1;
+  a.nchunks = a.NP * (unsigned)T;
+  a.fN = make_fastdiv((unsigned)N); a.fNP = make_fastdiv(a.NP);
+  long slabs = 2L * marl_wgrad_slabs(M);
+  if (slabs > (long)a.nchunks) slabs = a.nchunks;
+  const int KT = (K + 15) / 16;
+  const int KTT = KT <= 6 ? 6 : KT <= 10 ? 10 : 14;
+  const void* fn = KTT == 6 ? (const void*)wgrad_tall_kernel_x6<6, 3> : KTT == 10 ? (const void*)wgrad_tall_kernel_x6<10, 5>
+                   : a.x.k0 > 192 ? (const void*)wgrad_tall_kernel_x6<14, 7> : (const void*)wgrad_tall_kernel_x6<14, 6>;
+  const size_t lds = (size_t)2 * 3 * TCH * (KTT + 1) * 16 * 2 + 8 * TCH * (sizeof(long) + 2 * sizeof(int));
+  hipStream_t s = (hipStream_t)stream;
+  hipError_t e = hipFuncSetAttribute(fn, hipFuncAttributeMaxDynamicSharedMemorySize, (int)lds);
+  if (e != hipSuccess) return (int)e;
+  void* kargs[] = {(void*)&a};
+  e = hipLaunchKernel(fn, dim3((unsigned)slabs), dim3(512), kargs, lds, s);
+  if (e != hipSuccess) return (int)e;
+  MARL_CHECK_LAUNCH();
+  WredArgs r;
+  r.ws = ws; r.dW = dW; r.lddw = lddw; r.db = db; r.N = 64; r.K = K; r.slabs = (int)slabs; r.groups = 1; r.gs_dw = 0; r.gs_db = 0;
+  const long total = 64L * (K + 1);
+  hipLaunchKernelGGL(wgrad_reduce_kernel, dim3((unsigned)((total + 63) / 64)), dim3(64 * RSG), 0, s, r);
+  MARL_CHECK_LAUNCH();
+  return 0;
+}
diff --git a/marl_amd/csrc/optim.hip b/marl_amd/csrc/optim.hip
--- a/marl_amd/csrc/optim.hip
+++ b/marl_amd/csrc/optim.hip
@@ -98,13 +98,14 @@
   return 0;
 }
 
-static MarlSwitches g_switches = {1, 1, 4, 1, 1, 0, 1};
+static MarlSwitches g_switches = {1, 1, 4, 1, 1, 0, 1, 1};
 extern "C" const MarlSwitches* marl_switches(void) { return &g_switches; }
 static int* switch_slot(const char* name) {
   if (!name) return nullptr;
   struct { const char* n; int* p; } tab[] = {{"fwd_xs", &g_switches.fwd_xs}, {"fwd_w2l", &g_switches.fwd_w2l},
                                              {"bwd_pipe_max_rt", &g_switches.bwd_pipe_max_rt}, {"wgrad_tall", &g_switches.wgrad_tall},
-                                             {"wide_res", &g_switches.wide_res}, {"rollout_v1", &g_switches.rollout_v1}, {"unroll_r6", &g_switches.unroll_r6}};
+                                             {"wide_res", &g_switches.wide_res}, {"rollout_v1", &g_switches.rollout_v1}, {"unroll_r6", &g_switches.unroll_r6},
+                                             {"fc1_x6", &g_switches.fc1_x6}};
   for (auto& t : tab)
     if (!strcmp(t.n, name)) return t.p;
   return nullptr;
diff --git a/marl_amd/experiments.py b/marl_amd/experiments.py
--- a/marl_amd/experiments.py
+++ b/marl_amd/experiments.py
@@ -4,7 +4,8 @@
 import os
 import warnings
 
-LIB_DEFAULTS = {"fwd_xs": 1, "fwd_w2l": 1, "bwd_pipe_max_rt": 4, "wgrad_tall": 1, "wide_res": 1, "rollout_v1": 0, "unroll_r6": 1}
+LIB_DEFAULTS = {"fwd_xs": 1, "fwd_w2l": 1, "bwd_pipe_max_rt": 4, "wgrad_tall": 1, "wide_res": 1, "rollout_v1": 0, "unroll_r6": 1,
+                "fc1_x6": 1}
 HOST_DEFAULTS = {"no_pair": 0, "no_chain": 0, "chain_split": None, "mlp3_keep": 1, "x6_bwd_min_wg": 1, "force_reducer": 0}
 
 
diff --git a/marl_amd/ops.py b/marl_amd/ops.py
--- a/marl_amd/ops.py
+++ b/marl_amd/ops.py
@@ -112,8 +112,34 @@
           "marl_linear")
 
 
-def linear_wgrad(dY, x, dW, db, M, N, K, Yact=None, grp=None, lddw=None, bf16=False):
-    lib = _lib.load()
+def linear_wgrad_x6t_supported(x, B, T, N, K):
+    return bool(_lib.load().marl_linear_wgrad_x6t_supported(C.byref(x), B, T, N, K))
+
+
+def dxp_tiled_numel(B, T, N):
+    return _lib.load().marl_agent_bwd_x6_dxp_tiled_bytes(B, T, N) // 4
+
+
+def dxp_untile(dxp_tiled, B, T, N, H=64):
+    R = B * N
+    nt = (R + 15) // 16
+    t = dxp_tiled.reshape(-1)[:T * nt * 1024].reshape(T, nt, 4, 4, 16, 4)
+    rows = t.permute(0, 1, 3, 5, 2, 4).reshape(T, nt * 16, H)[:, :R]
+    return rows.reshape(T, B, N, H).permute(1, 0, 2, 3).contiguous()
+
+
+def linear_wgrad(dY, x, dW, db, M, N, K, Yact=None, grp=None, lddw=None, bf16=False, *, g_tiled=None, btn=None):
+    lib = _lib.load()
+    if g_tiled is not None:
+        B_, T_, N_ = btn
+        assert dY is None and Yact is None and grp is None and not bf16 and N == 64 and M == B_ * T_ * N_
+        assert src_width(x) == K, (src_width(x), K)
+        ws = WS.get("wgrad", lib.marl_linear_wgrad_workspace(M, N, K, 1), g_tiled.device)
+        if lddw is None:
+            lddw = dW.stride(0) if dW.dim() == 2 else K
+        check(lib.marl_linear_wgrad_x6t(_p(_f32(g_tiled)), C.byref(x), _p(_f32(dW)), lddw, _p(db), B_, T_, N_, K, _p(ws),
+                                        ws.numel() * 4, _stream()), "marl_linear_wgrad_x6t")
+        return
     flags = 1 if bf16 else 0
     g = grp.groups if grp is not None else 1
     nbytes = lib.marl_linear_wgrad_workspace(M, N, K, g)
@@ -208,7 +234,7 @@
 
 
 def agent_unroll_bwd(w, dq, dhs, saved, hs, dxp, dh0, grads, B, T, N, A, dq_idx=None, dq_val=None, dq_idx2=None,
-                     dq_val2=None, dq_gdiv=1, x6=False):
+                     dq_val2=None, dq_gdiv=1, x6=False, *, dxp_tiled=None):
     lib = _lib.load()
     g = MarlAgentGrads()
     g.w_ih, g.w_hh = grads["rnn.weight_ih"].data_ptr(), grads["rnn.weight_hh"].data_ptr()
@@ -223,10 +249,17 @@
             assert dq_val2 is not None and dq_idx2.is_contiguous() and dq_val2.is_contiguous()
             _i32(dq_idx2); _f32(dq_val2)
         ws = WS.get("agent_bwd_x6", lib.marl_agent_bwd_x6_workspace(B, N, A), saved.device)
+        if dxp_tiled is not None:
+            check(lib.marl_agent_unroll_bwd_x6_tiled(C.byref(w), _p(dq_idx), _p(dq_val), _p(dq_idx2), _p(dq_val2), int(dq_gdiv),
+                                                     _p(dhs), _p(_f32(saved)), _p(dxp), _p(_f32(dxp_tiled)), _p(dh0), C.byref(g),
+                                                     _p(ws), ws.numel() * 4, B, T, N, A, _stream()),
+                  "marl_agent_unroll_bwd_x6_tiled")
+            return
         check(lib.marl_agent_unroll_bwd_x6(C.byref(w), _p(dq_idx), _p(dq_val), _p(dq_idx2), _p(dq_val2), int(dq_gdiv), _p(dhs),
                                            _p(_f32(saved)), _p(_f32(dxp)), _p(dh0), C.byref(g), _p(ws), ws.numel() * 4, B, T, N, A,
                                            _stream()), "marl_agent_unroll_bwd_x6")
         return
+    assert dxp_tiled is None, "the tiled dxp is an output of the split BPTT only"
     ws = WS.get("agent_bwd", lib.marl_agent_bwd_workspace(B, N, A), saved.device)
     if dq_idx is not None:
         assert dq is None and dq_val is not None and dq_idx.is_contiguous() and dq_val.is_contiguous()
```

New measurement: 74.24 million (median of 6 runs). No clear change (+1.0%).
